# NeSC-IV/sage-icp

Measured on AMD Instinct MI355X. Metric: ICP frames/sec (120k-pt scan vs 1M-pt map), higher is better.
Workload: dtype f64

## Files before the change

### include/sageicp.h

```cpp
#ifndef SAGEICP_H_
#define SAGEICP_H_

#include <stddef.h>
#include <stdint.h>

#ifdef __cplusplus
extern "C" {
#endif

#define SAGEICP_OK 0
#define SAGEICP_ERR_INVALID (-1)
#define SAGEICP_ERR_NO_DEVICE (-2)
#define SAGEICP_ERR_HIP (-3)
#define SAGEICP_ERR_RCCL (-4)
#define SAGEICP_ERR_CAPACITY (-5)

typedef struct sageicp_map sageicp_map;
typedef struct sageicp_frame sageicp_frame;
typedef struct sageicp_comm sageicp_comm;

#define SAGEICP_ABI_VERSION 4

typedef struct sageicp_stats {
    int32_t iterations;
// ... 140 lines not shown
int sageicp_cluster_emission_order(const uint32_t *sizes, uint64_t n, uint32_t *order_out);

int sageicp_deskew_scan(const double *frame_xyzl, const double *timestamps, uint64_t n,
                        const double start_pose[7], const double finish_pose[7],
                        double *out_xyzl, int device);

typedef struct sageicp_pipeline sageicp_pipeline;
typedef struct sageicp_pipeline_config {
    double voxel_size_map, max_range, min_range, label_max_range, local_map_range;
    int basic_points_per_voxel, critical_points_per_voxel;
    const int *basic_parts_labels;
    int n_basic_parts_labels;
    double min_motion_th, initial_threshold, sem_th;
    int n_groups;
    const int *group_label_counts;
    const int *group_labels;
    const double *group_voxel_size;
    int device;
    int map_update_on_device;
} sageicp_pipeline_config;

sageicp_pipeline *sageicp_pipeline_create(const sageicp_pipeline_config *config);
void sageicp_pipeline_destroy(sageicp_pipeline *p);
int sageicp_pipeline_register_frame(sageicp_pipeline *p, const double *frame_xyzl, uint64_t n,
                                    double pose_out[7], double *icp_seconds, double *total_seconds,
                                    uint64_t *n_source, sageicp_stats *stats );
int sageicp_pipeline_prefetch(sageicp_pipeline *p, const double *next_frame_xyzl, uint64_t n);
int sageicp_pipeline_prefetch_wait(sageicp_pipeline *p);
int sageicp_pipeline_prefetch_cancel(sageicp_pipeline *p);
int sageicp_pipeline_set_dynamic_vehicle_filter(sageicp_pipeline *p, int enable, double dy_th,
                                                int dynamic_vehicle_voxid, const int *landmark_labels,
                                                int n_landmark);
int sageicp_pipeline_dynamic_filter_info(const sageicp_pipeline *p, sageicp_dynfilter_info *info);
int sageicp_pipeline_set_deskew(sageicp_pipeline *p, int enable);
int sageicp_pipeline_register_frame_timestamps(sageicp_pipeline *p, const double *frame_xyzl,
                                               const double *timestamps, uint64_t n, double pose_out[7],
                                               double *icp_seconds, double *total_seconds, uint64_t *n_source,
                                               sageicp_stats *stats );
int sageicp_pipeline_deskew_info(const sageicp_pipeline *p, int *applied, double delta_out[6]);

#define SAGEICP_DTYPE_FLOAT32 1
#define SAGEICP_DTYPE_FLOAT64 2
#define SAGEICP_DTYPE_UINT8 3
#define SAGEICP_DTYPE_INT32 4
#define SAGEICP_DTYPE_INT64 5
typedef struct sageicp_device_frame {
    const void *xyz;
    uint64_t xyz_stride;
    int32_t xyz_dtype;
    int32_t label_dtype;
    const void *label;
    uint64_t label_stride;
    uint64_t n;
} sageicp_device_frame;
int sageicp_pipeline_register_frame_device(sageicp_pipeline *p, const sageicp_device_frame *frame,
                                           const double *timestamps ,
                                           void *stream , double pose_out[7],
                                           double *icp_seconds, double *total_seconds, uint64_t *n_source,
                                           sageicp_stats *stats );
sageicp_frame *sageicp_frame_from_device(const sageicp_map *map, const sageicp_device_frame *frame,
                                         void *stream );

typedef struct sageicp_device_points {
    void *xyz;
    uint64_t xyz_stride;
    int32_t xyz_dtype;
    int32_t label_dtype;
    void *label;
    uint64_t label_stride;
    uint64_t cap;
} sageicp_device_points;
int sageicp_pipeline_source(const sageicp_pipeline *p, double *out_xyzl, uint64_t cap, uint64_t *n_out);
int sageicp_pipeline_source_device(const sageicp_pipeline *p, const sageicp_device_points *dst,
                                   void *stream , uint64_t *n_out);
int sageicp_map_pointcloud_device(const sageicp_map *m, const sageicp_device_points *dst,
                                  void *stream , uint64_t *n_out);
int sageicp_get_correspondences_device(const sageicp_map *map, const sageicp_device_frame *frame,
                                       const double pose[7] ,
                                       double max_correspondence_distance, double sem_th,
                                       const sageicp_device_points *src_out ,
                                       const sageicp_device_points *tgt_out ,
                                       int64_t *query_idx_out , uint64_t idx_cap,
                                       void *stream , uint64_t *n_out);

typedef struct sageicp_quality {
    double fitness, rmse, step_norm;
    double sum_r2, sum_w, sum_w_r2;
    double step[6];
    double JTr[6];
    double JTJ[36];
    double info[36];
    double covariance[36];
    double covariance_pose[36];
    double class_sum_r2[256];
    double other_sum_r2;
    uint64_t n_queries, n_pairs;
    uint64_t pairs_same_label, pairs_unlabelled, pairs_cross_label;
    uint64_t other_queries, other_pairs;
    uint32_t class_queries[256];
    uint32_t class_pairs[256];
    int32_t valid, covariance_valid;
} sageicp_quality;
int sageicp_registration_quality(const sageicp_map *map, const double *xyzl, uint64_t n,
                                 const double pose[7] , double max_correspondence_distance,
                                 double kernel, double sem_th, sageicp_quality *out);
int sageicp_registration_quality_device(const sageicp_map *map, const sageicp_device_frame *frame,
                                        const double pose[7] , double max_correspondence_distance,
                                        double kernel, double sem_th, void *stream ,
                                        sageicp_quality *out);
int sageicp_pipeline_set_quality(sageicp_pipeline *p, int enable);
int sageicp_pipeline_quality(const sageicp_pipeline *p, sageicp_quality *out);

typedef struct sageicp_pose_score {
    double score;
    double fitness, rmse, step_norm;
    double sum_r2, sum_w, sum_w_r2;
    double step[6], JTr[6], JTJ[36];
    uint64_t n_queries, n_pairs, pairs_same_label, pairs_unlabelled, pairs_cross_label;
    int32_t valid, step_valid;
} sageicp_pose_score;
int sageicp_score_poses(const sageicp_map *map, const double *xyzl, uint64_t n,
                        const double *poses , uint64_t k,
                        double max_correspondence_distance, double kernel, double sem_th,
                        sageicp_pose_score *out );
int sageicp_score_poses_device(const sageicp_map *map, const sageicp_device_frame *frame,
                               const double *poses , uint64_t k,
                               double max_correspondence_distance, double kernel, double sem_th,
                               void *stream , sageicp_pose_score *out);

typedef struct sageicp_relocalize_params {
    double xy_extent, xy_step, z_extent, z_step;
    double yaw_extent, yaw_step;
    uint32_t refine_top, reserved;
    double max_correspondence_distance, kernel, sem_th;
} sageicp_relocalize_params;
typedef struct sageicp_relocalize_info {
    uint64_t candidates, best_candidate;
    double best_candidate_score;
    uint32_t refined, winner_rank;
    int32_t iterations, converged;
    double us_score, us_refine, us_wall;
} sageicp_relocalize_info;
int sageicp_relocalize_candidates(const double prior[7], const sageicp_relocalize_params *params,
                                  double *poses_out , uint64_t cap, uint64_t *k_out);
int sageicp_relocalize(const sageicp_map *map, const double *xyzl, uint64_t n, const double prior[7],
                       const sageicp_relocalize_params *params, double pose_out[7],
                       sageicp_quality *quality_out , sageicp_relocalize_info *info );
int sageicp_relocalize_device(const sageicp_map *map, const sageicp_device_frame *frame, const double prior[7],
                              const sageicp_relocalize_params *params, void *stream, double pose_out[7],
                              sageicp_quality *quality_out, sageicp_relocalize_info *info);

int sageicp_pipeline_reinitialize(sageicp_pipeline *p);
uint64_t sageicp_pipeline_num_poses(const sageicp_pipeline *p);
int sageicp_pipeline_pose(const sageicp_pipeline *p, uint64_t index, double pose_out[7]);
const sageicp_map *sageicp_pipeline_local_map(const sageicp_pipeline *p);

typedef struct sageicp_occupancy_params {
    double bounds[3][2];
    int32_t occ_h, occ_w;
    double overlap_th;
} sageicp_occupancy_params;
typedef struct sageicp_key_frame_info {
    int32_t enabled;
    int32_t is_key_frame;
    double overlap;
    uint64_t key_frame_index;
// ... 93 lines not shown
```

### sage-icp_amd/__init__.py

```python
import ctypes as C
import os
import sys

import numpy as np

_HERE = os.path.dirname(os.path.abspath(__file__))
SQNORM3_ORDER = 0 if os.environ.get("SAGE_SQNORM3_ORDER", "2") == "0" else 2
if os.environ.get("SAGE_SQNORM3_ORDER", "2") not in ("0", "2"):
    import warnings
    warnings.warn("SAGE_SQNORM3_ORDER=%r: only the builds 0 and 2 exist — using 2" % os.environ["SAGE_SQNORM3_ORDER"])
LIB_PATH = os.path.join(_HERE, "libsageicp_hip.v0.so" if SQNORM3_ORDER == 0 else "libsageicp_hip.so")
if os.environ.get("SAGEICP_VARIANT_LIB"):
    LIB_PATH = os.path.abspath(os.environ["SAGEICP_VARIANT_LIB"])

_dp = C.POINTER(C.c_double)
_u64p = C.POINTER(C.c_uint64)
_i64p = C.POINTER(C.c_int64)
_u8p = C.POINTER(C.c_uint8)

ABI_VERSION = 4
ERR_INVALID, ERR_NO_DEVICE, ERR_HIP, ERR_RCCL, ERR_CAPACITY = -1, -2, -3, -4, -5
UNIQUE_ID_BYTES = 128
P2P_HANDLE_BYTES = 64

# ... 192 lines not shown
def occupancy_params(bounds=KEY_FRAME_BOUNDS, occ_size=KEY_FRAME_OCC_SIZE, overlap=KEY_FRAME_OVERLAP):
    b = [[float(v) for v in ax] for ax in bounds]
    if len(b) != 3 or any(len(ax) != 2 for ax in b):
        raise ValueError("bounds are ((x_lo, x_hi), (y_lo, y_hi), (z_lo, z_hi))")
    h, w = (int(v) for v in occ_size)
    p = OccupancyParams()
    for a in range(3):
        p.bounds[a][0], p.bounds[a][1] = b[a]
    p.occ_h, p.occ_w, p.overlap_th = h, w, float(overlap)
    return p


KITTI_VOXEL_LABELS = [[40, 44, 48, 49], [50, 51, 52], [70, 72], [60, 71, 80, 81, 99], [0],
                      [10, 11, 13, 15, 16, 18, 20]]
KITTI_VOXEL_SIZE = [0.6, 1.0, 0.9, 0.8, 1.0, 0.6]


def make_pipeline_config(voxel_size_map=0.8, max_range=100.0, min_range=5.0, label_max_range=50.0,
                         local_map_range=100.0, basic=20, critical=20,
                         basic_parts_labels=(40, 44, 48, 49, 50, 70, 72), min_motion_th=0.1,
                         initial_threshold=2.0, sem_th=0.05, voxel_labels=None, voxel_size=None,
                         device=0, map_update_on_device=True, dynamic_vehicle_filter=False,
                         dynamic_vehicle_filter_th=0.5, dynamic_vehicle_voxid=5, dynamic_remove_lankmark=(44, 48),
                         deskew=False):
    voxel_labels = KITTI_VOXEL_LABELS if voxel_labels is None else voxel_labels
    voxel_size = KITTI_VOXEL_SIZE if voxel_size is None else voxel_size
    assert len(voxel_labels) == len(voxel_size)
    keep = {}
    keep["basic"] = (C.c_int * len(basic_parts_labels))(*basic_parts_labels)
    keep["counts"] = (C.c_int * len(voxel_labels))(*[len(g) for g in voxel_labels])
    flat = [l for g in voxel_labels for l in g]
    keep["labels"] = (C.c_int * len(flat))(*flat)
    keep["sizes"] = (C.c_double * len(voxel_size))(*voxel_size)
    cfg = PipelineConfig(voxel_size_map, max_range, min_range, label_max_range, local_map_range,
                         basic, critical, keep["basic"], len(basic_parts_labels), min_motion_th,
                         initial_threshold, sem_th, len(voxel_labels), keep["counts"],
                         keep["labels"], keep["sizes"], device, 1 if map_update_on_device else 0)
    cfg._keep = keep
    cfg._dynamic = dict(enable=bool(dynamic_vehicle_filter), dy_th=float(dynamic_vehicle_filter_th),
                        voxid=int(dynamic_vehicle_voxid), landmarks=tuple(dynamic_remove_lankmark))
    cfg._deskew = bool(deskew)
    return cfg


_SIGNATURES = [
    ("sageicp_abi_version", C.c_int, []),
    ("sageicp_last_error", C.c_char_p, []),
    ("sageicp_device_count", C.c_int, []),
    ("sageicp_set_profiling", None, [C.c_int]),
    ("sageicp_set_counting", None, [C.c_int]),
    ("sageicp_reload_env", None, []),
    ("sageicp_map_loop_status", C.c_int, [C.c_void_p, C.c_void_p]),
    ("sageicp_set_downsample_order", None, [C.c_int]),
    ("sageicp_robin_iteration_order", C.c_int, [C.c_void_p, C.c_uint64, C.c_void_p]),
    ("sageicp_robin_sweep", C.c_int, [C.c_void_p, C.c_uint64, C.c_void_p, C.c_int, C.c_void_p, _u64p, C.c_void_p, _u64p]),
    ("sageicp_map_create", C.c_void_p,
     [C.c_double, C.c_double, C.c_int, C.c_int, C.POINTER(C.c_int), C.c_int, C.c_int]),
    ("sageicp_map_destroy", None, [C.c_void_p]),
    ("sageicp_map_set_devices", C.c_int, [C.c_void_p, C.POINTER(C.c_int), C.c_int]),
    ("sageicp_map_num_devices", C.c_int, [C.c_void_p]),
    ("sageicp_map_set_reference_order", C.c_int, [C.c_void_p, C.c_int]),
    ("sageicp_map_reference_order", C.c_int, [C.c_void_p]),
    ("sageicp_map_clone", C.c_void_p, [C.c_void_p]),
    ("sageicp_map_clear", C.c_int, [C.c_void_p]),
    ("sageicp_map_empty", C.c_int, [C.c_void_p]),
    ("sageicp_map_size", C.c_uint64, [C.c_void_p]),
    ("sageicp_map_num_voxels", C.c_uint64, [C.c_void_p]),
    ("sageicp_map_add_points", C.c_int, [C.c_void_p, _dp, C.c_uint64]),
    ("sageicp_map_remove_far", C.c_int, [C.c_void_p, _dp]),
    ("sageicp_map_update", C.c_int, [C.c_void_p, _dp, C.c_uint64, _dp]),
    ("sageicp_map_update_pose", C.c_int, [C.c_void_p, _dp, C.c_uint64, _dp]),
    ("sageicp_map_update_pose_device", C.c_int, [C.c_void_p, _dp, C.c_uint64, _dp]),
    ("sageicp_map_pointcloud", C.c_uint64, [C.c_void_p, _dp, C.c_uint64]),
    ("sageicp_map_resident", C.c_int, [C.c_void_p]),
    ("sageicp_map_point_slots", C.c_uint64, [C.c_void_p]),
    ("sageicp_voxel_hash", C.c_uint32, [C.c_int32, C.c_int32, C.c_int32]),
    ("sageicp_map_table_stats", C.c_int, [C.c_void_p, _u64p]),
    ("sageicp_map_sync", C.c_int, [C.c_void_p]),
    ("sageicp_get_correspondences", C.c_int,
     [C.c_void_p, _dp, C.c_uint64, C.c_double, C.c_double, _dp, _dp, _u64p, _i64p]),
    ("sageicp_get_correspondences_device", C.c_int,
     [C.c_void_p, C.POINTER(DeviceFrame), _dp, C.c_double, C.c_double, C.POINTER(DevicePoints), C.POINTER(DevicePoints),
      C.c_void_p, C.c_uint64, C.c_void_p, _u64p]),
    ("sageicp_registration_quality", C.c_int,
     [C.c_void_p, _dp, C.c_uint64, _dp, C.c_double, C.c_double, C.c_double, C.POINTER(Quality)]),
    ("sageicp_registration_quality_device", C.c_int,
     [C.c_void_p, C.POINTER(DeviceFrame), _dp, C.c_double, C.c_double, C.c_double, C.c_void_p, C.POINTER(Quality)]),
    ("sageicp_pipeline_set_quality", C.c_int, [C.c_void_p, C.c_int]),
    ("sageicp_pipeline_quality", C.c_int, [C.c_void_p, C.POINTER(Quality)]),
    ("sageicp_score_poses", C.c_int,
     [C.c_void_p, _dp, C.c_uint64, _dp, C.c_uint64, C.c_double, C.c_double, C.c_double, C.c_void_p]),
    ("sageicp_score_poses_device", C.c_int,
     [C.c_void_p, C.POINTER(DeviceFrame), _dp, C.c_uint64, C.c_double, C.c_double, C.c_double, C.c_void_p, C.c_void_p]),
    ("sageicp_relocalize_candidates", C.c_int, [_dp, C.POINTER(RelocalizeParams), _dp, C.c_uint64, _u64p]),
    ("sageicp_relocalize", C.c_int,
     [C.c_void_p, _dp, C.c_uint64, _dp, C.POINTER(RelocalizeParams), _dp, C.POINTER(Quality), C.POINTER(RelocalizeInfo)]),
    ("sageicp_relocalize_device", C.c_int,
     [C.c_void_p, C.POINTER(DeviceFrame), _dp, C.POINTER(RelocalizeParams), C.c_void_p, _dp, C.POINTER(Quality),
      C.POINTER(RelocalizeInfo)]),
    ("sageicp_align_clouds", C.c_int, [_dp, _dp, C.c_uint64, C.c_double, _dp, _dp, _dp, C.c_int]),
    ("sageicp_transform_points", C.c_int, [_dp, _dp, C.c_uint64, C.c_int]),
    ("sageicp_register_frame", C.c_int,
     [C.c_void_p, _dp, C.c_uint64, _dp, C.c_double, C.c_double, C.c_double, _dp,
      C.POINTER(Stats)]),
    ("sageicp_frame_upload", C.c_void_p, [C.c_void_p, _dp, C.c_uint64]),
    ("sageicp_frame_destroy", None, [C.c_void_p]),
    ("sageicp_register_frame_resident", C.c_int,
     [C.c_void_p, C.c_void_p, _dp, C.c_double, C.c_double, C.c_double, C.c_void_p, _dp,
      C.POINTER(Stats)]),
    ("sageicp_comm_unique_id", C.c_int, [_u8p]),
    ("sageicp_comm_create", C.c_void_p, [_u8p, C.c_int, C.c_int, C.c_int]),
    ("sageicp_comm_create_local", C.c_void_p, [C.c_int, C.c_int, C.c_int]),
    ("sageicp_comm_p2p_export", C.c_int, [C.c_void_p, C.POINTER(C.c_uint8)]),
    ("sageicp_comm_p2p_connect", C.c_int, [C.c_void_p, C.POINTER(C.c_uint8)]),
    ("sageicp_comm_p2p_enable", C.c_int, [C.c_void_p, C.c_int]),
    ("sageicp_comm_p2p_enabled", C.c_int, [C.c_void_p]),
    ("sageicp_comm_describe", C.c_int, [C.c_void_p, C.POINTER(CommInfo)]),
    ("sageicp_comm_destroy", None, [C.c_void_p]),
    ("sageicp_preprocess", C.c_int,
     [_dp, C.c_uint64, C.c_double, C.c_double, C.c_double, _dp, _u64p, C.c_int]),
    ("sageicp_voxel_downsample", C.c_int,
     [_dp, C.c_uint64, C.c_int, C.POINTER(C.c_int), C.POINTER(C.c_int), C.POINTER(C.c_double),
      C.c_double, _dp, _u64p, C.c_int]),
    ("sageicp_preprocess_dynamic", C.c_int,
     [_dp, C.c_uint64, C.c_double, C.c_double, C.c_double, C.c_double, C.POINTER(C.c_int), C.c_int,
      C.POINTER(C.c_int), C.c_int, _dp, _u64p, C.POINTER(DynFilterInfo), C.c_int]),
    ("sageicp_cluster_emission_order", C.c_int, [C.c_void_p, C.c_uint64, C.c_void_p]),
    ("sageicp_pipeline_set_dynamic_vehicle_filter", C.c_int,
     [C.c_void_p, C.c_int, C.c_double, C.c_int, C.POINTER(C.c_int), C.c_int]),
    ("sageicp_pipeline_dynamic_filter_info", C.c_int, [C.c_void_p, C.POINTER(DynFilterInfo)]),
    ("sageicp_deskew_scan", C.c_int, [_dp, _dp, C.c_uint64, _dp, _dp, _dp, C.c_int]),
    ("sageicp_pipeline_set_deskew", C.c_int, [C.c_void_p, C.c_int]),
    ("sageicp_pipeline_register_frame_timestamps", C.c_int,
     [C.c_void_p, _dp, _dp, C.c_uint64, _dp, _dp, _dp, _u64p, C.POINTER(Stats)]),
    ("sageicp_pipeline_deskew_info", C.c_int, [C.c_void_p, C.POINTER(C.c_int), _dp]),
    ("sageicp_pipeline_register_frame_device", C.c_int,
     [C.c_void_p, C.POINTER(DeviceFrame), C.c_void_p, C.c_void_p, _dp, _dp, _dp, _u64p, C.POINTER(Stats)]),
    ("sageicp_frame_from_device", C.c_void_p, [C.c_void_p, C.POINTER(DeviceFrame), C.c_void_p]),
    ("sageicp_pipeline_source", C.c_int, [C.c_void_p, _dp, C.c_uint64, _u64p]),
    ("sageicp_pipeline_source_device", C.c_int, [C.c_void_p, C.POINTER(DevicePoints), C.c_void_p, _u64p]),
    ("sageicp_map_pointcloud_device", C.c_int, [C.c_void_p, C.POINTER(DevicePoints), C.c_void_p, _u64p]),
    ("sageicp_pipeline_set_key_frames", C.c_int, [C.c_void_p, C.c_int, C.POINTER(OccupancyParams)]),
    ("sageicp_pipeline_key_frame_reset", C.c_int, [C.c_void_p]),
    ("sageicp_pipeline_key_frame_info", C.c_int, [C.c_void_p, C.POINTER(KeyFrameInfo)]),
    ("sageicp_pipeline_key_frame_grid", C.c_int, [C.c_void_p, C.c_void_p, C.c_uint64]),
    ("sageicp_pipeline_key_frame_grid_device", C.c_int, [C.c_void_p, C.c_void_p, C.c_uint64, C.c_void_p]),
    ("sageicp_occupancy_grid", C.c_int, [_dp, C.c_uint64, _dp, C.POINTER(OccupancyParams), C.c_void_p, C.c_int]),
    ("sageicp_occupancy_grid_device", C.c_int,
     [C.POINTER(DeviceFrame), _dp, C.POINTER(OccupancyParams), C.c_void_p, C.c_void_p]),
    ("sageicp_pipeline_register_frame_msg", C.c_int,
     [C.c_void_p, C.c_void_p, C.c_uint64, C.c_uint64, C.POINTER(MsgLayout), _dp, _dp, _dp, _u64p, C.POINTER(Stats)]),
    ("sageicp_pipeline_register_frame_msg_device", C.c_int,
     [C.c_void_p, C.c_void_p, C.c_uint64, C.c_uint64, C.POINTER(MsgLayout), C.c_void_p, _dp, _dp, _dp, _u64p,
      C.POINTER(Stats)]),
    ("sageicp_msg_output_fields", C.c_uint32, [C.POINTER(MsgField), C.c_uint32]),
    ("sageicp_pipeline_source_msg", C.c_int, [C.c_void_p, C.POINTER(MsgColors), C.c_void_p, C.c_uint64, _u64p]),
    ("sageicp_pipeline_source_msg_device", C.c_int,
     [C.c_void_p, C.POINTER(MsgColors), C.c_void_p, C.c_uint64, C.c_void_p, _u64p]),
    ("sageicp_map_pointcloud_msg", C.c_int, [C.c_void_p, C.POINTER(MsgColors), C.c_void_p, C.c_uint64, _u64p]),
    ("sageicp_map_pointcloud_msg_device", C.c_int,
     [C.c_void_p, C.POINTER(MsgColors), C.c_void_p, C.c_uint64, C.c_void_p, _u64p]),
    ("sageicp_map_set_archive", C.c_int, [C.c_void_p, C.c_int, C.c_uint64]),
    ("sageicp_map_archive_info", C.c_int, [C.c_void_p, C.POINTER(ArchiveInfo)]),
    ("sageicp_map_archive_clear", C.c_int, [C.c_void_p]),
    ("sageicp_map_archive_voxels", C.c_int, [C.c_void_p, C.c_uint64, C.c_void_p, C.c_uint64, _u64p]),
    ("sageicp_map_archive_rows", C.c_int, [C.c_void_p, C.c_int, C.c_uint64, _dp, C.c_uint64, _u64p]),
# ... 656 lines not shown
            _check(lib().sageicp_relocalize_device(self._h, C.byref(f), pr, C.byref(params), stream,
                                                   pose.ctypes.data_as(_dp), C.byref(q), C.byref(info)))
            return pose, q, info.as_dict()
        if labels is not None:
            raise ValueError("labels= is for a frame that is a torch tensor on a GPU")
        pts, fp = _d(pts)
        _check(lib().sageicp_relocalize(self._h, fp, pts.reshape(-1, 4).shape[0], pr, C.byref(params),
                                        pose.ctypes.data_as(_dp), C.byref(q), C.byref(info)))
        return pose, q, info.as_dict()

    def _correspondences_device(self, pts, max_dist, th, with_index, labels, pose, dtype):
        f, stream = _device_rows(DeviceFrame, pts, labels, self.device, _FRAME_WORDS)
        pp = None
        if pose is not None:
            pose_a, pp = _d(pose)
            if pose_a.size != 7:
                raise ValueError("a pose is (qx, qy, qz, qw, tx, ty, tz)")
        import torch
        dt = torch.float64 if dtype is None else dtype
        if dt not in (torch.float32, torch.float64):
            raise ValueError("dtype= is torch.float32 or torch.float64, not %s" % (dt,))
        n = int(f.n)
        src = torch.empty((n, 4), dtype=dt, device=pts.device)
        tgt = torch.empty((n, 4), dtype=dt, device=pts.device)
        idx = torch.empty(n, dtype=torch.int64, device=pts.device) if with_index else None
        ds, _ = _device_rows(DevicePoints, src, None, self.device, _OUT_WORDS, distinct=True)
        dg, _ = _device_rows(DevicePoints, tgt, None, self.device, _OUT_WORDS, distinct=True)
        nout = C.c_uint64(0)
        _check(lib().sageicp_get_correspondences_device(
            self._h, C.byref(f), pp, max_dist, th, C.byref(ds), C.byref(dg),
            (idx.data_ptr() or None) if with_index else None, n, stream, C.byref(nout)))
        k = nout.value
        return (src[:k], tgt[:k], idx[:k]) if with_index else (src[:k], tgt[:k])


def _relocalize_params(xy, z, yaw, refine_top=0, max_correspondence_distance=0.0, kernel=1.0, sem_th=0.0):
    p = RelocalizeParams()
    (p.xy_extent, p.xy_step), (p.z_extent, p.z_step), (p.yaw_extent, p.yaw_step) = xy, z, yaw
    p.refine_top = refine_top
    p.max_correspondence_distance, p.kernel, p.sem_th = max_correspondence_distance, kernel, sem_th
    return p


def relocalize_candidates(prior, xy=(0, 0), z=(0, 0), yaw=(0, 0), cap=None):
    prior_a, pr = _d(prior)
    if prior_a.size != 7:
        raise ValueError("a pose is (qx, qy, qz, qw, tx, ty, tz)")
    params = _relocalize_params(xy, z, yaw)
    k = C.c_uint64(0)
    if cap is None:
        _check(lib().sageicp_relocalize_candidates(pr, C.byref(params), None, 0, C.byref(k)))
    rows = k.value if cap is None else int(cap)
    out = np.empty((rows, 7))
    _check(lib().sageicp_relocalize_candidates(pr, C.byref(params), out.ctypes.data_as(_dp), rows, C.byref(k)))
    return out if cap is None else (out[:min(rows, k.value)], k.value)


def register_frame(frame, voxel_map, initial_guess, max_correspondence_distance, kernel, sem_th,
                   comm=None, return_stats=False):
    init, ip = _d(initial_guess)
    out = np.empty(7)
    st = Stats()
    if isinstance(frame, Frame):
        _check(lib().sageicp_register_frame_resident(
            voxel_map._h, frame._h, ip, max_correspondence_distance, kernel, sem_th,
            comm._h if comm is not None else None, out.ctypes.data_as(_dp), C.byref(st)))
    else:
        if comm is not None:
            raise ValueError("sharded registration needs a resident Frame")
        pts, pp = _d(frame)
        _check(lib().sageicp_register_frame(
            voxel_map._h, pp, pts.reshape(-1, 4).shape[0], ip, max_correspondence_distance,
            kernel, sem_th, out.ctypes.data_as(_dp), C.byref(st)))
    return (out, st) if return_stats else out


def transform_points(pose, pts, device=0):
    T, tp = _d(pose)
    out = np.array(pts, dtype=np.float64, order="C", copy=True).reshape(-1, 4)
    _check(lib().sageicp_transform_points(tp, out.ctypes.data_as(_dp), out.shape[0], device))
    return out


def occupancy_grid(frame, bounds=KEY_FRAME_BOUNDS, occ_size=KEY_FRAME_OCC_SIZE, pose=None, device=0, labels=None):
    params = occupancy_params(bounds, occ_size, 0.0)
    out = np.zeros((params.occ_h, params.occ_w), dtype=np.uint8)
    pp = None
    if pose is not None:
        pose_a, pp = _d(pose)
        if pose_a.size != 7:
            raise ValueError("a pose is (qx, qy, qz, qw, tx, ty, tz)")
    if _is_device_tensor(frame):
        f, stream = _device_rows(DeviceFrame, frame, labels, frame.device.index, _FRAME_WORDS)
        _check(lib().sageicp_occupancy_grid_device(C.byref(f), pp, C.byref(params), out.ctypes.data_as(C.c_void_p),
                                                   stream))
        return out
    if labels is not None:
        raise ValueError("labels= is for a frame that is a torch tensor on a GPU")
    pts, fp = _d(frame)
    _check(lib().sageicp_occupancy_grid(fp, pts.reshape(-1, 4).shape[0], pp, C.byref(params),
                                        out.ctypes.data_as(C.c_void_p), device))
    return out


def align_clouds(src, tgt, kernel, device=0):
    src, sp = _d(src)
    tgt, gp = _d(tgt)
    T = np.empty(7)
    JTJ = np.empty(36)
    JTr = np.empty(6)
    _check(lib().sageicp_align_clouds(sp, gp, src.reshape(-1, 4).shape[0], kernel,
                                      T.ctypes.data_as(_dp), JTJ.ctypes.data_as(_dp),
                                      JTr.ctypes.data_as(_dp), device))
    return T, JTJ.reshape(6, 6), JTr


class SageICP:

    def __init__(self, config=None, **kw):
        self.config = config if config is not None else make_pipeline_config(**kw)
        self._h = lib().sageicp_pipeline_create(C.byref(self.config))
        if not self._h:
            raise SageIcpError(ERR_INVALID, (lib().sageicp_last_error() or b"").decode())
        self._deskew_on = False
        dyn = getattr(self.config, "_dynamic", None)
        if dyn and dyn["enable"]:
            self.set_dynamic_vehicle_filter(True, dyn["dy_th"], dyn["voxid"], dyn["landmarks"])
        if getattr(self.config, "_deskew", False):
            self.set_deskew(True)

    def set_deskew(self, enable=True):
        _check(lib().sageicp_pipeline_set_deskew(self._h, 1 if enable else 0))
        self._deskew_on = bool(enable)
        if enable:
            self._announced = ()

    def deskew_info(self):
        applied = C.c_int(0)
        delta = np.zeros(6)
        _check(lib().sageicp_pipeline_deskew_info(self._h, C.byref(applied), delta.ctypes.data_as(_dp)))
        return bool(applied.value), delta

    def set_dynamic_vehicle_filter(self, enable=True, dy_th=0.5, voxid=5, landmark_labels=(44, 48)):
        lm = (C.c_int * max(len(landmark_labels), 1))(*landmark_labels)
        _check(lib().sageicp_pipeline_set_dynamic_vehicle_filter(self._h, 1 if enable else 0, dy_th, voxid, lm,
                                                                 len(landmark_labels)))

    def set_quality(self, enable=True):
        _check(lib().sageicp_pipeline_set_quality(self._h, 1 if enable else 0))

    def quality(self):
        q = Quality()
        _check(lib().sageicp_pipeline_quality(self._h, C.byref(q)))
        return q

    def set_key_frames(self, enable=True, bounds=KEY_FRAME_BOUNDS, occ_size=KEY_FRAME_OCC_SIZE, overlap=KEY_FRAME_OVERLAP):
        params = occupancy_params(bounds, occ_size, overlap) if enable else None
        _check(lib().sageicp_pipeline_set_key_frames(self._h, 1 if enable else 0,
                                                     C.byref(params) if params is not None else None))
        self._occ_size = (params.occ_h, params.occ_w) if enable else None

    def key_frame_info(self):
        info = KeyFrameInfo()
        _check(lib().sageicp_pipeline_key_frame_info(self._h, C.byref(info)))
        return info.as_dict()

# ... 313 lines not shown
```

### sage-icp_amd/build.py

```python
import concurrent.futures
import hashlib
import os
import subprocess

HERE = os.path.dirname(os.path.abspath(__file__))
SOURCES = ["csrc/kernels.hip", "csrc/sort.hip", "csrc/preprocess.hip", "csrc/dyn_filter.hip", "csrc/deskew.hip",
           "csrc/ingest.hip", "csrc/egress.hip", "csrc/msg.hip", "csrc/keyframe.hip", "csrc/map_update.hip",
           "csrc/map_device.hip", "csrc/capi_run.hip", "csrc/prep.hip", "csrc/capi.hip", "csrc/capi_pipeline.hip",
           "csrc/capi_outputs.hip", "csrc/caller_mem.hip", "csrc/correspond.hip", "csrc/quality.hip", "csrc/score.hip",
           "csrc/capi_query.hip", "csrc/capi_relocalize.hip", "csrc/archive.hip", "csrc/capi_archive.hip"]
HEADERS = ["csrc/kernels.h", "csrc/dev_buffer.h", "csrc/sageicp_types.h", "csrc/se3_math.h", "csrc/host_map.hpp", "csrc/pipeline.hpp", "csrc/map_update.h", "csrc/egress.h", "csrc/msg.h", "csrc/metrics.hpp", "csrc/robin_order.hpp", "csrc/capi_internal.h", "csrc/prep.h", "csrc/prefetch.h", "csrc/dyn_rules.h", "csrc/probes.h", "csrc/icp_body.h", "csrc/row_shift.h", "csrc/fin_kernel.h", "csrc/loop_kernel.h", "csrc/loop_deal.h", "csrc/caller_mem.h", "csrc/outputs.h", "csrc/map_device.h", "csrc/replay_pool.h", "csrc/correspond.h", "csrc/quality.h", "csrc/score.h", "csrc/accept.h", "csrc/archive.h", "csrc/query.h",
           "../include/sageicp.h"]
OUT = os.path.join(HERE, "libsageicp_hip.so")
OBJ_DIR = os.path.join(HERE, "build")

FLAGS = ["--offload-arch=gfx950", "-O3", "-std=c++17", "-fPIC", "-ffp-contract=off",
         "-Wall", "-Wextra"]


def _stamp(extra):
    h = hashlib.sha1(" ".join(FLAGS + list(extra)).encode())
    for f in HEADERS:
        with open(os.path.join(HERE, f), "rb") as fh:
            h.update(fh.read())
    return h.hexdigest()[:16]


def needs_build():
    if not os.path.exists(OUT):
        return True
    t = os.path.getmtime(OUT)
    return any(os.path.getmtime(os.path.join(HERE, f)) > t for f in SOURCES + HEADERS)


def _prune(keep, newest=6):
    import shutil
    dirs = [os.path.join(OBJ_DIR, d) for d in os.listdir(OBJ_DIR)]
    dirs = sorted((d for d in dirs if os.path.isdir(d) and d != keep), key=os.path.getmtime, reverse=True)
    for d in dirs[newest - 1:]:
        shutil.rmtree(d, ignore_errors=True)


def build(force=False, verbose=False, out=OUT, defines=(), jobs=None):
    if not force and out == OUT and not defines and not needs_build():
        return out
    hipcc = os.environ.get("HIPCC", "/opt/rocm/bin/hipcc")
    extra = ["-D" + d for d in defines]
    tag = _stamp(extra)
    odir = os.path.join(OBJ_DIR, tag)
    os.makedirs(odir, exist_ok=True)
    _prune(keep=odir)

    def compile_one(src):
        path = os.path.join(HERE, src)
        obj = os.path.join(odir, os.path.basename(src) + ".o")
        if os.path.exists(obj) and os.path.getmtime(obj) >= os.path.getmtime(path):
            return obj
        cmd = [hipcc] + FLAGS + extra + ["-c", path, "-o", obj]
        if verbose:
            print(" ".join(cmd))
        subprocess.check_call(cmd)
        return obj

    with concurrent.futures.ThreadPoolExecutor(max_workers=jobs or min(len(SOURCES), os.cpu_count() or 1)) as ex:
        objs = list(ex.map(compile_one, SOURCES))
    cmd = [hipcc, "--offload-arch=gfx950", "-shared", "-fPIC"] + objs + ["-o", out, "-ldl", "-lpthread"]
    if verbose:
        print(" ".join(cmd))
    subprocess.check_call(cmd)
    return out


def build_sqnorm3_variant(force=False, verbose=False):
    out = os.path.join(HERE, "libsageicp_hip.v0.so")
    if not force and os.path.exists(out):
        t = os.path.getmtime(out)
        if not any(os.path.getmtime(os.path.join(HERE, f)) > t for f in SOURCES + HEADERS):
            return out
    return build(force=True, verbose=verbose, out=out, defines=("SAGE_SQNORM3_ORDER=0",))


PROBE_DEFINES = ("SAGE_NN_TIMING", "SAGE_LOOP_TIMING", "SAGE_GN_TIMING", "SAGE_ICP_DELAY_PROBE", "SAGE_LOOP_INGRID")


def compile_probe_variants(jobs=None):
    hipcc = os.environ.get("HIPCC", "/opt/rocm/bin/hipcc")
    src = os.path.join(HERE, "csrc/kernels.hip")

    def one(d):
        r = subprocess.run([hipcc] + FLAGS + ["-D" + d, "--cuda-device-only", "-c", src, "-o", os.devnull],
                           capture_output=True, text=True)
        return d, (r.stderr if r.returncode else "")

    with concurrent.futures.ThreadPoolExecutor(max_workers=jobs or min(len(PROBE_DEFINES), os.cpu_count() or 1)) as ex:
# ... 9 lines not shown
```

### sage-icp_amd/csrc/capi_internal.h

```cpp
#pragma once

#include <dlfcn.h>
#include <hip/hip_runtime.h>
#include <rccl/rccl.h>

#include <atomic>
#include <chrono>
#include <cmath>
#include <cstdio>
#include <cstdlib>
#include <cfloat>
#include <limits>
#include <memory>
#include <cstring>
#include <map>
#include <array>
#include <string>
#include <utility>
#include <vector>

#include "../../include/sageicp.h"
#include "dev_buffer.h"
#include "dyn_rules.h"
#include "host_map.hpp"
// ... 39 lines not shown
inline int icp_lw(uint64_t n, bool sparse_voxels) {
    const int e = env_int("SAGEICP_LW", -1);
    if (e >= 0) return e > 4 ? 4 : e;
    if (n >= (sparse_voxels ? 150000u : 400000u)) return 1;
    if (n >= (sparse_voxels ? 60000u : 110000u)) return 2;
    if (n >= (sparse_voxels ? 4096u : 20000u)) return 3;
    return 4;
}


inline int fail(int code, const std::string &msg) {
    g_err = msg;
    return code;
}

#define HIPCHK(expr)                                                                      \
    do {                                                                                  \
        hipError_t _e = (expr);                                                           \
        if (_e != hipSuccess)                                                             \
            return fail(SAGEICP_ERR_HIP, std::string(#expr) + ": " + hipGetErrorString(_e)); \
    } while (0)

inline int require_device() {
    int count = 0;
    if (hipGetDeviceCount(&count) != hipSuccess || count <= 0)
        return fail(SAGEICP_ERR_NO_DEVICE, "no HIP device visible (gfx950 required; no CPU fallback)");
    return SAGEICP_OK;
}
inline int require_device(int device) {
    if (int rc = require_device()) return rc;
    if (device < 0 || device >= sageicp_device_count()) return fail(SAGEICP_ERR_INVALID, "device ordinal out of range");
    return SAGEICP_OK;
}

inline int stream_after_caller(OwnedEvent &ev, hipStream_t caller, hipStream_t ours) {
    if (!ev) HIPCHK(ev.create(hipEventDisableTiming));
    HIPCHK(hipEventRecord(ev.get(), caller));
    HIPCHK(hipStreamWaitEvent(ours, ev.get(), 0));
    return SAGEICP_OK;
}

inline bool finite_n(const double *v, uint64_t n) {
    for (uint64_t i = 0; i < n; ++i)
        if (!std::isfinite(v[i])) return false;
    return true;
}

inline double now_us() {
    using namespace std::chrono;
    return duration<double, std::micro>(steady_clock::now().time_since_epoch()).count();
}

constexpr int kChunkMax = 16;

struct Scratch {
    int device = -1;
    OwnedStream stream;
    DevBuf<Point4> d_frame, d_tgt;
    DevBuf<int32_t> d_nn;
    DevBuf<Point4> d_sorted;
    DevBuf<uint32_t> d_keys, d_vals;
    DevBuf<unsigned char> d_sort_temp;
    size_t sort_cap = 0;
    DevBuf<uint32_t> d_rows;
    DevBuf<uint2> d_prev;
    DevBuf<uint32_t> d_work;
    DevBuf<double> d_partials;
    DevBuf<long long> d_acc;
    DevBuf<LoopShared> d_loop;
    unsigned long long go_word = 0;
    OwnedStream stream2;
    std::vector<uint32_t> cu_mask;
    OwnedEvent ev_solve;
    unsigned long long loop_epoch = 0;
    int num_cus = 0;
    int cu_share_i = 0, cu_share_k = 1;
    int loop_cooldown = 0;
    int loop_derate = 0;
    uint64_t calls_single_launch = 0, calls_per_iteration = 0, calls_chained = 0;
    uint32_t loop_timeouts = 0;
    int last_fallback = 0;
    DevBuf<unsigned long long> d_cand;
    DevBuf<IcpState> d_state;
    PinnedBuf<IcpState> h_state;
    PinnedBuf<IcpProgress, hipHostMallocMapped | hipHostMallocCoherent> h_prog;
    IcpProgress *d_prog = nullptr;
    std::vector<OwnedEvent> events;
    DevBuf<int32_t> d_by_query;
    DevBuf<uint32_t> d_corr_counts;
    DevBuf<unsigned long long> d_corr_words;
    PinnedBuf<unsigned long long> h_corr_words;
    DevBuf<double> d_qual_slabs;
    DevBuf<QualityRaw> d_qual_raw;
    PinnedBuf<QualityRaw> h_qual_raw;
    DevBuf<Point4> d_score_frame, d_score_rows;
    DevBuf<int32_t> d_score_by_query;
    DevBuf<double> d_score_slabs;
    DevBuf<ScorePose> d_score_poses;
    PinnedBuf<ScorePose> h_score_poses;
    DevBuf<ScoreRaw> d_score_raw;
    PinnedBuf<ScoreRaw> h_score_raw;

    ~Scratch() { wait(); }
    void wait() const {
        if (!stream) return;
        (void)hipSetDevice(device);
        (void)hipStreamSynchronize(stream.get());
        if (stream2) (void)hipStreamSynchronize(stream2.get());
    }

    int init(int dev) {
        if (stream) return SAGEICP_OK;
        if (int rc = require_device(dev)) return rc;
        device = dev;
        HIPCHK(hipSetDevice(device));
        {
            int cus = 0;
            if (hipDeviceGetAttribute(&cus, hipDeviceAttributeMultiprocessorCount, device) == hipSuccess) num_cus = cus;
        }
        if (cu_share_k <= 1) {
            if (const char *e = env_cached("SAGEICP_CU_SHARE")) {
                int i = 0, k = 1;
                if (std::sscanf(e, "%d/%d", &i, &k) == 2 && k >= 1 && k <= 16 && i >= 0 && i < k) {
                    cu_share_i = i;
                    cu_share_k = k;
                }
            }
        }
        if (cu_share_k > 1 && num_cus >= 8 * cu_share_k) {
            const int per = num_cus / cu_share_k, lo = cu_share_i * per;
            std::vector<uint32_t> mask((num_cus + 31) / 32, 0u);
            for (int c = lo; c < lo + per; ++c) mask[c / 32] |= 1u << (c % 32);
            HIPCHK(stream.create(static_cast<uint32_t>(mask.size()), mask.data()));
            cu_mask = mask;
            num_cus = per;
        } else {
            cu_share_i = 0;
            cu_share_k = 1;
            HIPCHK(stream.create());
        }
        HIPCHK(d_state.reserve(1));
        HIPCHK(d_acc.reserve(kAccReplicas * kAccWords));
        HIPCHK(d_loop.reserve(1));
        HIPCHK(hipMemset(d_loop.data(), 0, sizeof(LoopShared)));

        HIPCHK(h_state.reserve(1));
        HIPCHK(h_prog.reserve(1));
        HIPCHK(hipHostGetDevicePointer(reinterpret_cast<void **>(&d_prog), h_prog.data(), 0));
        return SAGEICP_OK;
    }
    int loop_streams() {
        if (stream2) return SAGEICP_OK;
        HIPCHK(hipSetDevice(device));
        if (!cu_mask.empty()) HIPCHK(stream2.create(static_cast<uint32_t>(cu_mask.size()), cu_mask.data()));
        else {
            int least = 0, greatest = 0;
            (void)hipDeviceGetStreamPriorityRange(&least, &greatest);
            if (stream2.create(greatest) != hipSuccess) {
                (void)hipGetLastError();
                HIPCHK(stream2.create());
            }
        }
        HIPCHK(ev_solve.create(hipEventDisableTiming));
        return SAGEICP_OK;
    }
    int reserve_frame(size_t n) {
        if (n > d_frame.capacity()) HIPCHK(d_frame.reserve(n + n / 4 + 1024));
        return SAGEICP_OK;
    }
    int reserve_tgt(size_t n) {
        if (n > d_tgt.capacity()) HIPCHK(d_tgt.reserve(n + n / 4 + 1024));
        return SAGEICP_OK;
    }
    int reserve_nn(size_t n) {
        if (n > d_nn.capacity()) HIPCHK(d_nn.reserve(n + n / 4 + 1024));
        return SAGEICP_OK;
    }
    int reserve_sort(size_t n) {
        if (n <= sort_cap) return SAGEICP_OK;
        sort_cap = 0;
        const size_t cap = n + n / 4 + 1024;
        HIPCHK(d_sorted.reserve(cap));
        HIPCHK(d_rows.reserve(cap * kRowWords));
        HIPCHK(d_prev.reserve(cap));
#ifdef SAGE_NN_TIMING
        HIPCHK(d_work.reserve(cap));
#endif
        HIPCHK(d_cand.reserve(2 * cap));
        HIPCHK(d_keys.reserve(2 * cap));
        HIPCHK(d_vals.reserve(2 * cap));
        HIPCHK(d_sort_temp.reserve(sort_temp_bytes(static_cast<int>(cap))));
        sort_cap = cap;
        return SAGEICP_OK;
    }
    int reserve_correspond(size_t n) {
        if (n > d_by_query.capacity()) HIPCHK(d_by_query.reserve(n + n / 4 + 1024));
        const size_t words = 2 * static_cast<size_t>(correspond_blocks(static_cast<int>(n)));
        if (words > d_corr_counts.capacity()) HIPCHK(d_corr_counts.reserve(words + words / 4 + 16));
        if (!d_corr_words) HIPCHK(d_corr_words.reserve(2));
        if (!h_corr_words) HIPCHK(h_corr_words.reserve(2));
        return SAGEICP_OK;
    }
    int reserve_quality(size_t n) {
        if (n > d_by_query.capacity()) HIPCHK(d_by_query.reserve(n + n / 4 + 1024));
        if (!d_qual_slabs) HIPCHK(d_qual_slabs.reserve(kQualSlabDoubles));
        if (!d_qual_raw) HIPCHK(d_qual_raw.reserve(1));
        if (!h_qual_raw) HIPCHK(h_qual_raw.reserve(1));
        return SAGEICP_OK;
    }
    int reserve_score_frame(size_t n) {
        if (n > d_score_frame.capacity()) HIPCHK(d_score_frame.reserve(n + n / 4 + 1024));
        return SAGEICP_OK;
    }
    int reserve_score(size_t n, size_t kc) {
        const size_t rows = n * kc, slabs = score_slab_doubles(static_cast<int>(n), static_cast<uint32_t>(kc));
        if (rows > d_score_rows.capacity()) HIPCHK(d_score_rows.reserve(rows + rows / 4 + 1024));
        if (rows > d_score_by_query.capacity()) HIPCHK(d_score_by_query.reserve(rows + rows / 4 + 1024));
        if (slabs > d_score_slabs.capacity()) HIPCHK(d_score_slabs.reserve(slabs + slabs / 4 + 1024));
        if (kc > d_score_poses.capacity()) HIPCHK(d_score_poses.reserve(kc + kc / 4 + 16));
        if (kc > h_score_poses.capacity()) HIPCHK(h_score_poses.reserve(kc + kc / 4 + 16));
        if (kc > d_score_raw.capacity()) HIPCHK(d_score_raw.reserve(kc + kc / 4 + 16));
        if (kc > h_score_raw.capacity()) HIPCHK(h_score_raw.reserve(kc + kc / 4 + 16));
        return SAGEICP_OK;
    }
    int reserve_partials(size_t blocks) {
        if (blocks > d_partials.capacity() / kNumSums) HIPCHK(d_partials.reserve((blocks + blocks / 4 + 256) * kNumSums));
        return SAGEICP_OK;
    }
    int reserve_events(size_t iterations) {
        while (events.size() < 5 * iterations) {
            OwnedEvent e;
// ... 9 lines not shown

#include "prep.h"

using namespace sageicp;

#include "caller_mem.h"
#include "map_device.h"
#include "archive.h"
#include "outputs.h"

struct sageicp_map {
    HostMap host;
    int device = 0;
    Scratch sc;
    sageicp_impl::MapDevice dev;
    sageicp_impl::OutputBuffers out;
    sageicp_impl::MapArchive arc;
    std::vector<sageicp_map *> replicas;
    std::vector<struct sageicp_comm *> ranks;
    bool replicas_diverged = false;

    bool resident() const { return dev.authority(); }
    bool empty() const { return counts().voxels == 0; }
    sageicp_impl::MapCounts counts() const {
        const bool on_device = dev.authority();
        const MapCounters &c = dev.ctr;
        sageicp_impl::MapCounts n;
        n.points = on_device ? c.total_points : host.total_points;
        n.voxels = on_device ? c.num_voxels : host.num_voxels;
        n.units_hi = on_device ? c.units_hi : host.units_hi;
        n.table_capacity = on_device ? dev.d_table.capacity() : host.table.size();
        n.used_slots = on_device ? c.used_slots : host.num_voxels;
        return n;
    }
    ~sageicp_map() { sc.wait(); }
};

inline sageicp_map &internal(const sageicp_map *m) { return *const_cast<sageicp_map *>(m); }

struct sageicp_frame {
    int device = 0;
    DevBuf<Point4> d;
    uint64_t n = 0;
};

struct sageicp_comm {
    ncclComm_t comm = nullptr;
    int rank = 0, nranks = 1, device = 0;
    bool p2p = false;
    bool poisoned = false;
    P2pBlock *my_block = nullptr;
    P2pBlock *blocks[kMaxRanks] = {};
    DevBuf<unsigned long long> d_exchanges;
    bool peer_mapped = false;
    bool device_shared = false;
};

namespace sageicp_impl {
struct Rccl {
    void *h = nullptr;
    ncclResult_t (*GetUniqueId)(ncclUniqueId *) = nullptr;
    ncclResult_t (*CommInitRank)(ncclComm_t *, int, ncclUniqueId, int) = nullptr;
    ncclResult_t (*CommDestroy)(ncclComm_t) = nullptr;
    ncclResult_t (*AllReduce)(const void *, void *, size_t, ncclDataType_t, ncclRedOp_t, ncclComm_t,
                              hipStream_t) = nullptr;
    const char *(*GetErrorString)(ncclResult_t) = nullptr;
    ncclResult_t (*CommCount)(const ncclComm_t, int *) = nullptr;
    ncclResult_t (*CommUserRank)(const ncclComm_t, int *) = nullptr;
};
extern Rccl g_rccl;
int load_rccl();
int register_resident(sageicp_map &m, const Point4 *d_frame, uint64_t n, int device, const double init[7],
                      double max_dist, double kernel, double sem_th, sageicp_comm *comm, double pose_out[7],
                      sageicp_stats *stats);
int refresh_mirror(sageicp_map &m);
int ensure_host(sageicp_map &m);
int device_update(sageicp_map &m, const double *xyzl, uint64_t n, const double pose[7], const Point4 *d_points = nullptr);
bool all_finite(const double *xyzl, uint64_t n);
void host_remove_far(sageicp_map &m, const double origin[3]);
void identity_pose(double T[7]);
void fill_state(IcpState *st, const double init[7]);
double accept_threshold(double max_dist);
bool sparse_voxels(const sageicp_map &m);
bool wants_filter(const sageicp_map &m, uint64_t n, double sem_th);
IcpParams icp_params(const sageicp_map &m, const Point4 *d_queries, uint64_t n, double sem_th, int lw, int acc_shift);
int run_icp(sageicp_map &m, const Point4 *d_frame, uint64_t n, const double init[7], double max_dist, double kernel,
            double sem_th, sageicp_comm *comm, double out[7], sageicp_stats *stats, double us_upload, double t_begin);
int device_update_all(sageicp_map &m, const double *xyzl, uint64_t n, const double pose[7], const Point4 *d_points);
int register_sharded(sageicp_map &m, const double *h_frame, const Point4 *d_frame, uint64_t n, const double init[7],
                     double max_dist, double kernel, double sem_th, double pose_out[7], sageicp_stats *stats, double t0);
}
using namespace sageicp_impl;
```

### sage-icp_amd/csrc/capi_query.hip

```cpp
#include "query.h"

namespace sageicp_impl {

int QueryCall::stage(const FrameSource &src, Point4 *d_dst) {
    if (src.kind == FrameSource::kHostRows) {
        HIPCHK(hipMemcpyAsync(d_dst, src.rows, src.n * sizeof(Point4), hipMemcpyHostToDevice, stream()));
        return SAGEICP_OK;
    }
    if (src.kind != FrameSource::kDeviceFrame)
        return fail(SAGEICP_ERR_INVALID, std::string(who_) + ": host rows or a device frame");
    if (int rc = stream_after_caller(m.out.ev_caller, src.stream, stream())) return rc;
    launch_ingest(ingest_args(*src.frame), d_dst, stream());
    HIPCHK(hipGetLastError());
    return SAGEICP_OK;
}

int QueryCall::stage(const Point4 *d_rows, uint64_t n, Point4 *d_dst) {
    HIPCHK(hipMemcpyAsync(d_dst, d_rows, n * sizeof(Point4), hipMemcpyDeviceToDevice, stream()));
    return SAGEICP_OK;
}

int QueryCall::move(Point4 *d_rows, uint64_t n, const double *pose) {
    double I[7];
    identity_pose(I);
    fill_state(sc.h_state.data(), pose ? pose : I);
    HIPCHK(hipMemcpyAsync(sc.d_state.data(), sc.h_state.data(), sizeof(IcpState), hipMemcpyHostToDevice, stream()));
    if (pose) launch_tf(d_rows, static_cast<int>(n), sc.d_state.data(), stream());
    HIPCHK(hipGetLastError());
    return SAGEICP_OK;
}

int QueryCall::sort_and_search(const Point4 *d_rows, uint64_t n, double sem_th, bool read_verdict) {
    HIPCHK(sort_frame(d_rows, sc.d_sorted.data(), static_cast<int>(n), sc.d_state.data(), false, false,
                      m.host.voxel_size, sc.d_keys.data(), sc.d_vals.data(), sc.d_sort_temp.data(),
                      sc.d_sort_temp.capacity(), stream()));
    if (read_verdict) {
        HIPCHK(hipMemcpyAsync(sc.h_state.data(), sc.d_state.data(), sizeof(IcpState), hipMemcpyDeviceToHost, stream()));
        if (int rc = wait()) return rc;
        if (sc.h_state.data()->bad_input) return refuse_non_finite(who_, noun_);
    }
    const int lw = icp_lw(n, sparse_voxels(m));
    if (int rc = m.dev.ensure_cand(wants_filter(m, n, sem_th), stream())) return rc;
    const IcpParams ip = icp_params(m, sc.d_sorted.data(), n, sem_th, lw, 0);
    launch_rows(ip, stream());
    launch_icp(ip, lw, false, stream());
    HIPCHK(hipGetLastError());
    return SAGEICP_OK;
}

CorrespondArgs QueryCall::answers(uint64_t n, double max_dist, int32_t *d_by_query) const {
    CorrespondArgs a{};
    a.n = static_cast<int>(n);
    a.sorted = sc.d_sorted.data();
    a.perm = sc.d_vals.data() + n;
    a.nn = sc.d_nn.data();
    a.pts = m.dev.search_view().pts;
    a.accept_r2 = accept_threshold(max_dist);
    a.by_query = d_by_query;
    return a;
}

int QueryCall::accept(uint64_t n, double max_dist, int32_t *d_by_query) {
    launch_corr_flag(answers(n, max_dist, d_by_query), stream());
    HIPCHK(hipGetLastError());
    return SAGEICP_OK;
}

int refuse_non_finite(const char *who, const char *noun) {
    return fail(SAGEICP_ERR_INVALID,
                std::string(who) + ": a coordinate or label of a " + noun + " is not finite (NaN / Inf)");
}

int check_host_rows(const char *who, const double *xyzl, uint64_t n) {
    if (n && !xyzl) return fail(SAGEICP_ERR_INVALID, std::string(who) + ": xyzl is NULL");
    if (n > kMaxQueries) return fail(SAGEICP_ERR_INVALID, std::string(who) + ": too many rows (2^26 - 4 max)");
    if (!all_finite(xyzl, n)) return refuse_non_finite(who, "row");
    return SAGEICP_OK;
}

int check_device_source(const char *who, const sageicp_map *map, const sageicp_device_frame *frame, void *stream) {
    if (!frame) return fail(SAGEICP_ERR_INVALID, std::string(who) + ": frame is NULL");
    if (int rc = check_frame_layout(frame)) return rc;
    if (int rc = check_device_frame(frame, nullptr, stream, map->device)) return rc;
    return check_stream(stream, map->device);
}

static_assert(sizeof(sageicp_quality) == 5464, "sageicp_quality: doubles first, no padding (include/sageicp.h)");
static_assert(kQualClasses == 256, "the class tables of sageicp_quality");

constexpr double kQualPivotBound = 1.0 / 67108864.0;

bool quality_solve(const double JTJ[36], const double JTr[6], double sum_w_r2, uint64_t n_pairs, QualitySolve *o) {
    if (n_pairs < 3) return false;
    const double np = static_cast<double>(n_pairs);
    double L[6][6] = {};
    for (int j = 0; j < 6; ++j) {
        double d = JTJ[j * 6 + j];
        for (int k = 0; k < j; ++k) d -= L[j][k] * L[j][k];
        if (!(d > kQualPivotBound * JTJ[j * 6 + j]) || !std::isfinite(d)) return false;
        L[j][j] = std::sqrt(d);
        for (int i = j + 1; i < 6; ++i) {
            double v = JTJ[i * 6 + j];
            for (int k = 0; k < j; ++k) v -= L[i][k] * L[j][k];
            L[i][j] = v / L[j][j];
        }
    }
    double Li[6][6] = {};
    for (int j = 0; j < 6; ++j) {
        Li[j][j] = 1.0 / L[j][j];
        for (int i = j + 1; i < 6; ++i) {
            double v = 0.0;
            for (int k = j; k < i; ++k) v -= L[i][k] * Li[k][j];
            Li[i][j] = v / L[i][i];
        }
    }
    for (int i = 0; i < 6; ++i)
        for (int j = 0; j <= i; ++j) {
            double v = 0.0;
// ... 95 lines not shown
                          c.stream()));
    if ((rc = c.wait())) return rc;
    quality_finish(*sc.h_qual_raw.data(), n, pose, out);
    return SAGEICP_OK;
}

int quality_of_device_rows(sageicp_map &m, const Point4 *d_rows, uint64_t n, const double *pose, double max_dist,
                           double kernel, double sem_th, sageicp_quality *out) {
    QueryCall c(m, "RegistrationQuality");
    if (int rc = c.sc.reserve_frame(n)) return rc;
    if (int rc = c.stage(d_rows, n, c.sc.d_frame.data())) return rc;
    return quality_of_staged_rows(c, n, pose, max_dist, kernel, sem_th, out);
}

static int check_quality_args(const sageicp_map *map, const double *pose, double kernel, const sageicp_quality *out) {
    if (!map) return fail(SAGEICP_ERR_INVALID, "RegistrationQuality: map is NULL");
    if (!out) return fail(SAGEICP_ERR_INVALID, "RegistrationQuality: out is NULL");
    if (pose && !finite_n(pose, 7)) return fail(SAGEICP_ERR_INVALID, "RegistrationQuality: the pose is not finite");
    if (!(std::isfinite(kernel) && kernel > 0.0))
        return fail(SAGEICP_ERR_INVALID, "RegistrationQuality: kernel must be finite and above 0");
    return SAGEICP_OK;
}

static int registration_quality(const sageicp_map *map, const FrameSource &src, const double *pose, double max_dist,
                                double kernel, double sem_th, sageicp_quality *out) {
    std::memset(out, 0, sizeof(*out));
    sageicp_map &m = internal(map);
    if (src.n == 0 || m.empty()) return SAGEICP_OK;
    int rc = refresh_mirror(m);
    if (rc) return rc;
    QueryCall c(m, "RegistrationQuality");
    if ((rc = m.sc.reserve_frame(src.n))) return rc;
    if ((rc = c.stage(src, m.sc.d_frame.data()))) return rc;
    return quality_of_staged_rows(c, src.n, pose, max_dist, kernel, sem_th, out);
}

}

extern "C" {

int sageicp_get_correspondences(const sageicp_map *map, const double *q, uint64_t n, double max_dist,
                                double sem_th, double *src_out, double *tgt_out, uint64_t *n_out,
                                int64_t *query_idx_out) {
    if (!map || !n_out || (n && (!q || !src_out || !tgt_out)))
        return fail(SAGEICP_ERR_INVALID, "null argument");
    if (n > kMaxQueries) return fail(SAGEICP_ERR_INVALID, "too many queries (2^26 - 4 max)");
    *n_out = 0;
    if (!all_finite(q, n)) return refuse_non_finite("GetCorrespondences", "query");
    sageicp_map &m = internal(map);
    int rc = ensure_host(m);
    if (rc) return rc;
    if ((rc = refresh_mirror(m))) return rc;
    if (n == 0 || m.empty()) return SAGEICP_OK;
    QueryCall c(m, "GetCorrespondences", "query");
    Scratch &sc = m.sc;
    if ((rc = sc.reserve_frame(n))) return rc;
    if ((rc = sc.reserve_nn(n))) return rc;
    if ((rc = sc.reserve_sort(n))) return rc;
    if ((rc = c.stage(FrameSource::host_rows(q, n), sc.d_frame.data()))) return rc;
    if ((rc = c.move(sc.d_frame.data(), n, nullptr))) return rc;
    if ((rc = c.sort_and_search(sc.d_frame.data(), n, sem_th,  false))) return rc;
    std::vector<int32_t> idx(n);
    std::vector<uint32_t> perm(n);
    HIPCHK(hipMemcpyAsync(idx.data(), sc.d_nn.data(), n * sizeof(int32_t), hipMemcpyDeviceToHost, c.stream()));
    HIPCHK(hipMemcpyAsync(perm.data(), sc.d_vals.data() + n, n * sizeof(uint32_t), hipMemcpyDeviceToHost, c.stream()));
    if ((rc = c.wait())) return rc;
    std::vector<int32_t> by_query(n);
    for (uint64_t i = 0; i < n; ++i) by_query[perm[i]] = idx[i];
    uint64_t k = 0;
    for (uint64_t i = 0; i < n; ++i) {
        if (by_query[i] < 0) continue;
        const Point4 &t = m.host.pts[by_query[i]];
        const double dx = t.x - q[4 * i], dy = t.y - q[4 * i + 1], dz = t.z - q[4 * i + 2];
        if (!(std::sqrt(SAGE_SQNORM3_ACCEPT(dx * dx, dy * dy, dz * dz)) < max_dist)) continue;
        std::memcpy(src_out + 4 * k, q + 4 * i, 32);
        std::memcpy(tgt_out + 4 * k, &t, 32);
        if (query_idx_out) query_idx_out[k] = static_cast<int64_t>(i);
        ++k;
    }
    *n_out = k;
    return SAGEICP_OK;
}

int sageicp_get_correspondences_device(const sageicp_map *map, const sageicp_device_frame *frame, const double pose[7],
                                       double max_dist, double sem_th, const sageicp_device_points *src_out,
                                       const sageicp_device_points *tgt_out, int64_t *query_idx_out, uint64_t idx_cap,
                                       void *stream, uint64_t *n_out) {
    if (!map || !frame || !n_out) return fail(SAGEICP_ERR_INVALID, "null argument");
    int rc = check_frame_layout(frame);
    if (!rc && src_out) rc = check_points_layout(src_out);
    if (!rc && tgt_out) rc = check_points_layout(tgt_out);
    if (rc) return rc;
    if (pose && !finite_n(pose, 7)) return fail(SAGEICP_ERR_INVALID, "GetCorrespondences: the pose is not finite");
    {
        const uint64_t caps[3] = {src_out ? src_out->cap : 0, tgt_out ? tgt_out->cap : 0, idx_cap};
        const bool given[3] = {src_out != nullptr, tgt_out != nullptr, query_idx_out != nullptr};
        for (int a = 0; a < 3; ++a)
            for (int b = a + 1; b < 3; ++b)
                if (given[a] && given[b] && caps[a] != caps[b])
                    return fail(SAGEICP_ERR_INVALID, "GetCorrespondences: src_out->cap, tgt_out->cap and idx_cap of the "
                                                     "destinations given must be equal");
    }
    if (reinterpret_cast<uintptr_t>(query_idx_out) % 8)
        return fail(SAGEICP_ERR_INVALID, "GetCorrespondences: query_idx_out must be 8-byte aligned");
    CallerExtent ext[5];
    int n_ext = 0;
    int first_of_tgt = 0, first_of_idx = 0;
    if (src_out) n_ext += points_extents(*src_out, ext + n_ext);
    first_of_tgt = n_ext;
    if (tgt_out) n_ext += points_extents(*tgt_out, ext + n_ext);
    first_of_idx = n_ext;
    if (query_idx_out && idx_cap) {
        const char *p = reinterpret_cast<const char *>(query_idx_out);
        ext[n_ext++] = {p, p + idx_cap * sizeof(int64_t)};
    }
    for (int a = 0; a < n_ext; ++a)
        for (int b = a + 1; b < n_ext; ++b) {
            const bool same = (b < first_of_tgt) || (a >= first_of_tgt && b < first_of_idx);
            if (!same && ext[a].overlaps(ext[b]))
                return fail(SAGEICP_ERR_INVALID, "GetCorrespondences: src_out, tgt_out and query_idx_out must not overlap "
                                                 "each other");
        }
    if ((rc = check_device_frame(frame, nullptr, stream, map->device))) return rc;
    if (src_out && (rc = check_device_points(src_out, stream, map->device))) return rc;
    if (tgt_out && (rc = check_device_points(tgt_out, stream, map->device))) return rc;
    if (query_idx_out && idx_cap) {
        if ((rc = require_device())) return rc;
        if ((rc = check_extent(query_idx_out, idx_cap * sizeof(int64_t), map->device, "GetCorrespondences: query_idx_out")))
            return rc;
    }
    if ((rc = check_stream(stream, map->device))) return rc;
    sageicp_map &m = internal(map);
    const uint64_t n = frame->n;
    if (n == 0 || m.empty()) {
        *n_out = 0;
        return SAGEICP_OK;
    }
    if ((rc = refresh_mirror(m))) return rc;
    QueryCall c(m, "GetCorrespondences", "query");
    Scratch &sc = m.sc;
    if ((rc = sc.reserve_frame(n))) return rc;
    if ((rc = sc.reserve_nn(n))) return rc;
    if ((rc = sc.reserve_sort(n))) return rc;
    if ((rc = sc.reserve_correspond(n))) return rc;
    if ((rc = c.stage(FrameSource::device_frame(frame, nullptr, static_cast<hipStream_t>(stream)), sc.d_frame.data())))
        return rc;
    if ((rc = c.move(sc.d_frame.data(), n, pose))) return rc;
    if ((rc = c.sort_and_search(sc.d_frame.data(), n, sem_th))) return rc;
    HIPCHK(hipMemsetAsync(sc.d_corr_words.data(), 0, 2 * sizeof(unsigned long long), c.stream()));
    int *flags = reinterpret_cast<int *>(sc.d_corr_words.data() + 1);
    CorrespondArgs a = c.answers(n, max_dist, sc.d_by_query.data());
    a.frame = sc.d_frame.data();
    a.counts = sc.d_corr_counts.data();
    a.total = sc.d_corr_words.data();
    a.has_src = src_out != nullptr;
    a.has_tgt = tgt_out != nullptr;
    if (src_out) a.src = egress_args(*src_out, flags);
    if (tgt_out) a.tgt = egress_args(*tgt_out, flags);
    a.idx = reinterpret_cast<long long *>(query_idx_out);
    a.idx_cap = idx_cap;
    launch_correspond(a, c.stream());
    HIPCHK(hipGetLastError());
    unsigned long long *h_words = sc.h_corr_words.data();
    HIPCHK(hipMemcpyAsync(h_words, sc.d_corr_words.data(), 2 * sizeof(unsigned long long), hipMemcpyDeviceToHost,
                          c.stream()));
    if ((rc = c.wait())) return rc;
// ... 27 lines not shown
```

### sage-icp_amd/csrc/capi_run.hip

```cpp
#include "capi_internal.h"
#include "accept.h"

#include <condition_variable>
#include <mutex>
#include <thread>

namespace sageicp_impl {

Rccl g_rccl;
static std::mutex g_rccl_mu;


int load_rccl() {
    std::lock_guard<std::mutex> lk(g_rccl_mu);
    if (g_rccl.h) return SAGEICP_OK;
    const char *names[] = {"librccl.so.1", "librccl.so", "/opt/rocm/lib/librccl.so.1"};
    void *h = nullptr;
    for (const char *n : names) {
        h = dlopen(n, RTLD_NOW | RTLD_NOLOAD | RTLD_GLOBAL);
        if (h) break;
    }
    for (int i = 0; i < 3 && !h; ++i) h = dlopen(names[i], RTLD_NOW | RTLD_GLOBAL);
    if (!h) return fail(SAGEICP_ERR_RCCL, std::string("cannot load librccl: ") + dlerror());
    g_rccl.GetUniqueId = reinterpret_cast<decltype(g_rccl.GetUniqueId)>(dlsym(h, "ncclGetUniqueId"));
// ... 116 lines not shown
    if (mode == 0 || n == 0 || sc.num_cus < 8) return false;
    const bool sparse = sparse_voxels(m);
    const bool filter = wants_filter(m, n, sem_th);
    const uint64_t cus = static_cast<uint64_t>(sc.num_cus);
    const int env_nw = std::min(kLoopMaxWavesHost, std::max(0, env_int("SAGEICP_LOOP_WAVES", 0)));
    const int env_gpw = std::max(0, env_int("SAGEICP_LOOP_GPW", 0));
    auto groups_at = [n](int l) { return (n + (64u >> l) - 1) / (64u >> l); };
    auto slots = [&](int k) {
        const uint64_t a = static_cast<uint64_t>(k) * cus * 15 / 16;
        int less = 0;
        for (int sh = 1; sh < sc.cu_share_k; sh *= 2) ++less;
        return (less > 0 && k > less) ? std::min(a, static_cast<uint64_t>(k - less) * cus) : a;
    };
    auto round32 = [](uint64_t w) { return std::max<uint64_t>(32, (w + 31) / 32 * 32); };
    auto countable = [](uint64_t wgs, uint64_t gpw, int lw) {
        return wgs / kLoopReplicas <= 255 && (wgs / kLoopReplicas) * gpw * ((64u >> lw) / 4u) <= 8192;
    };
    auto one_pass = [&](int lw, int nw, LoopPlan *pl) {
        const uint64_t wgs = round32((groups_at(lw) + nw - 1) / nw);
        const size_t lds = loop_lds_bytes(lw, nw, nw);
        const int k = loop_wgs_per_cu(sc, lw, filter, nw, lds);
        if (k < 1 || wgs + 32ull * static_cast<uint64_t>(sc.loop_derate) > slots(k) || !countable(wgs, nw, lw)) return false;
        *pl = LoopPlan{lw, nw, nw, static_cast<int>(wgs), filter};
        return true;
    };
    auto multi_pass = [&](int lw, LoopPlan *pl) {
        const uint64_t groups = groups_at(lw);
        int best = -1;
        const int order[] = {4, 8, 7, 6, 5, 3, 2, 1};
        for (int nw : order) {
            if (env_nw && nw != env_nw) continue;
            if (!env_nw && nw < 4) continue;
            for (int k = SAGE_LOOP_OCC / ((nw + 3) / 4); k >= 1; --k) {
                if (static_cast<uint64_t>(k) * cus < 34) break;
                uint64_t cap = slots(k) / 32 * 32;
                cap = cap > 32ull * static_cast<uint64_t>(sc.loop_derate) ? cap - 32ull * static_cast<uint64_t>(sc.loop_derate) : 0;
                if (cap < 32) continue;
                if (const int e = env_int("SAGEICP_LOOP_MAX_WGS", 0)) cap = std::min<uint64_t>(cap, static_cast<uint64_t>(e) / 32 * 32);
                uint64_t gpw = env_gpw ? static_cast<uint64_t>(env_gpw) : (groups + cap - 1) / cap;
                const uint64_t wgs = env_gpw ? round32((groups + gpw - 1) / gpw) : std::min(cap, round32(groups));
                if (wgs > cap) continue;
                if (!env_gpw) gpw = (groups + wgs - 1) / wgs;
                const size_t lds = loop_lds_bytes(lw, nw, static_cast<int>(gpw));
                if (lds > 160 * 1024 || !countable(wgs, gpw, lw)) continue;
                if (loop_wgs_per_cu(sc, lw, filter, nw, lds) < k) continue;
                if (k * nw > best) {
                    best = k * nw;
                    *pl = LoopPlan{lw, nw, static_cast<int>(gpw), static_cast<int>(wgs), filter};
                }
                break;
            }
        }
        return best > 0;
    };
    const int forced = env_int("SAGEICP_LW", -1);
    int lw = forced >= 0 ? std::min(forced, 4) : icp_lw(n, sparse);
    if (lw < 1) return false;
    if (forced < 0 && !env_gpw) {
        const uint64_t few = 15 * cus;
        if (lw < 3 && groups_at(3) <= few) lw = 3;
        if (lw == 3 && !sparse && groups_at(4) <= few) lw = 4;
        const uint64_t resident_waves = 4ull * SAGE_LOOP_OCC * cus * 15 / 16;
        while (lw > 2 && groups_at(lw) > resident_waves * 4 / 5) --lw;
    }
    const bool dbg = env_int("SAGEICP_LOOP_DEBUG", 0) != 0;
    bool ok = !env_gpw && one_pass(lw, env_nw ? env_nw : 4, out);
    if (!ok) ok = multi_pass(lw, out);
    if (dbg) {
        if (ok)
            std::fprintf(stderr, "sageicp: one-launch loop for %llu queries: %d lanes/query, %d workgroups of %d waves, <= %d units of %d queries each, "
                                 "%zu B of LDS (%d workgroups per CU by the occupancy query, %d CUs)\n",
                         static_cast<unsigned long long>(n), 1 << out->lw, out->wgs, out->nw,
                         out->gpw, 64 >> out->lw, loop_lds_bytes(out->lw, out->nw, out->gpw),
                         loop_wgs_per_cu(sc, out->lw, filter, out->nw, loop_lds_bytes(out->lw, out->nw, out->gpw)), sc.num_cus);
        else
            std::fprintf(stderr, "sageicp: %llu queries at %d lanes/query do not fit the one-launch loop (7 waves x 4 workgroups "
                                 "of 36 KB per CU by the occupancy query: %d)\n",
                         static_cast<unsigned long long>(n), 1 << lw,
                         loop_wgs_per_cu(sc, lw, filter, 7, 36 * 1024));
    }
    return ok;
}

struct Attempt {
    int acc_shift = 0;
    int restarts = 0;
    bool no_loop = false;
    bool no_chain = false;
};

struct IcpCall {
    sageicp_map &m;
    const Point4 *d_frame;
    uint64_t n;
    const double *init;
    double max_dist, kernel, sem_th;
    sageicp_comm *comm;
    Scratch &sc;
    hipStream_t s;
    bool p2p, polled, prof, prof2, counting;
    int max_it;
    P2pParams xp;

    int constants(bool want_stats) {
        prof = g_profiling != 0;
        prof2 = g_profiling >= 2;
        p2p = comm && comm->p2p;
        if (comm && !p2p && !comm->comm)
            return fail(SAGEICP_ERR_INVALID, "communicator without RCCL needs a connected p2p exchange");
        polled = (!comm || p2p) && env_int("SAGEICP_CHUNKED", 0) == 0;
        max_it = std::min(kMaxIterations, std::max(1, env_int("SAGEICP_MAX_ITER", kMaxIterations)));
        counting = want_stats && g_counting != 0;
        xp.nranks = 1;
        if (!p2p) return SAGEICP_OK;
        xp.nranks = comm->nranks;
        xp.rank = comm->rank;
        for (int r = 0; r < comm->nranks; ++r) xp.block[r] = comm->blocks[r];
        xp.exchanges = comm->d_exchanges.data();
        xp.timeout_ticks = 100000000ull * static_cast<unsigned long long>(std::max(1, env_int("SAGEICP_P2P_TIMEOUT_S", 5)));
        if (const int ticks = env_int("SAGEICP_P2P_TIMEOUT_TICKS", 0))
            xp.timeout_ticks = static_cast<unsigned long long>(ticks);
        return SAGEICP_OK;
    }
    int start_state() const {
        fill_state(sc.h_state.data(), init);
        if (polled) {
            std::memset(sc.h_prog.data(), 0, sizeof(IcpProgress));
            sc.h_state.data()->progress = sc.d_prog;
        }
        HIPCHK(hipMemcpyAsync(sc.d_state.data(), sc.h_state.data(), sizeof(IcpState), hipMemcpyHostToDevice, s));
        return SAGEICP_OK;
    }
    int fetch_state(unsigned nwaves) const {
        if (counting) launch_sum_counters(sc.d_cand.data(), static_cast<int>(nwaves), sc.d_state.data(), s);
        HIPCHK(hipGetLastError());
        HIPCHK(hipMemcpyAsync(sc.h_state.data(), sc.d_state.data(), sizeof(IcpState), hipMemcpyDeviceToHost, s));
        HIPCHK(hipStreamSynchronize(s));
        return SAGEICP_OK;
    }
    int order_frame() const {
        if (n > 0 && n < static_cast<uint64_t>(std::max(0, env_int("SAGEICP_SORT_FROM", kSortFrameFrom))))
            HIPCHK(check_copy_frame(d_frame, sc.d_sorted.data(), static_cast<int>(n), sc.d_state.data(), comm == nullptr, s));
        else if (n > 0)
            HIPCHK(sort_frame(d_frame, sc.d_sorted.data(), static_cast<int>(n), sc.d_state.data(), true, comm == nullptr,
                              m.host.voxel_size, sc.d_keys.data(), sc.d_vals.data(), sc.d_sort_temp.data(),
                              sc.d_sort_temp.capacity(), s));
        return SAGEICP_OK;
    }
};

struct AttemptPlan {
    LoopPlan loop{};
    bool loop_shape = false, use_loop = false, chain = false;
    int lw = 0, chain_grid = 0;
    unsigned loop_waves = 0;
};
static AttemptPlan plan_attempt(const IcpCall &c, const Attempt &a) {
    Scratch &sc = c.sc;
    const sageicp_comm *comm = c.comm;
    const uint64_t n = c.n;
    AttemptPlan p;
    p.loop_shape = (!comm || (c.p2p && !comm->device_shared && env_int("SAGEICP_CHUNKED", 0) == 0)) &&
                   plan_loop(c.m, n, c.sem_th, &p.loop);
    p.lw = p.loop_shape ? p.loop.lw : icp_lw(n, sparse_voxels(c.m));
    p.use_loop = p.loop_shape && !a.no_loop;
    sc.last_fallback = !p.loop_shape ? SAGEICP_LOOP_FALLBACK_DOES_NOT_FIT : (a.no_loop ? SAGEICP_LOOP_FALLBACK_PEER : SAGEICP_LOOP_FALLBACK_NONE);
    if (p.use_loop && sc.loop_cooldown > 0) {
        --sc.loop_cooldown;
        p.use_loop = false;
        sc.last_fallback = SAGEICP_LOOP_FALLBACK_COOLDOWN;
    }
    p.loop_waves = p.use_loop ? static_cast<unsigned>((n + (64u >> p.loop.lw) - 1) / (64u >> p.loop.lw)) : 0u;
    p.chain_grid = n > 0 ? icp_blocks_for(static_cast<int>(n), p.lw) : 0;
    const bool chain_comm = comm && c.p2p && !comm->device_shared && env_int("SAGEICP_CHAIN_COMM", 0) != 0;
    p.chain = !p.loop_shape && (!comm || chain_comm) && c.polled && n > 0 &&
              p.chain_grid / kChainReplicas <= 255 && !a.no_chain && !c.prof2 && env_int("SAGEICP_CHAIN", 1) != 0;
    return p;
}

static bool solver_is_own_launch(const AttemptPlan &p) {
#ifdef SAGE_LOOP_INGRID
    return p.chain;
#else
    return p.chain || p.use_loop;
#endif
}

static LoopParams solver_params(const IcpCall &c, const AttemptPlan &p, double acc_unscale) {
    LoopParams L{};
    L.sh = c.sc.d_loop.data();
    L.st = c.sc.d_state.data();
    L.timeout_ticks = 100000ull * static_cast<unsigned long long>(std::max(1, env_int("SAGEICP_LOOP_TIMEOUT_MS", 50)));
    const int test_ticks = env_int("SAGEICP_LOOP_TIMEOUT_TICKS", 0);
    if (test_ticks) L.timeout_ticks = static_cast<unsigned long long>(test_ticks);
    if (p.chain) {
        L.wgs = p.chain_grid;
        L.copies = kChainReplicas;
        L.progress = c.sc.d_prog;
        L.count_timeout_ticks = std::max<unsigned long long>(L.timeout_ticks, 20ull * 100000ull) * 10ull;
    } else {
        L.nw = p.loop.nw; L.gpw = p.loop.gpw; L.wgs = p.loop.wgs;
        L.copies = kLoopReplicas;
        L.progress = nullptr;
        L.contiguous = env_int("SAGEICP_LOOP_CONTIGUOUS", 0) ? 1 : 0;
        const uint64_t qw = 64u >> p.loop.lw, groups = (c.n + qw - 1) / qw;
        for (int x = 0; x <= 8; ++x) L.xcd_first[x] = static_cast<uint32_t>(groups * x / 8);
        const uint64_t nwg = static_cast<uint64_t>(p.loop.wgs / 8);
        for (int x = 0; x < 8; ++x)
            if (L.contiguous == 1 && (L.xcd_first[x + 1] - L.xcd_first[x] + nwg - 1) / nwg > static_cast<uint64_t>(p.loop.gpw)) L.contiguous = 0;
        L.count_timeout_ticks = L.timeout_ticks;
        L.prio = std::min(3, std::max(0, env_int("SAGEICP_LOOP_PRIO", 3)));
        L.deal = std::min(2, std::max(0, env_int("SAGEICP_LOOP_DEAL", 1)));
    }
    if (c.comm) {
        L.shared_loop = 1;
        if (test_ticks == 0) L.timeout_ticks = std::max(L.timeout_ticks, c.xp.timeout_ticks + 100000000ull);
        if (env_int("SAGEICP_LOOP_COUNT_TIMEOUT_RANK", -1) == c.comm->rank)
            L.count_timeout_ticks = static_cast<unsigned long long>(std::max(1, env_int("SAGEICP_LOOP_COUNT_TIMEOUT_TICKS", 1)));
    }
    L.pose_map = std::min(2, std::max(0, env_int("SAGEICP_LOOP_POSE_MAP", 0)));
    L.max_iterations = c.max_it;
    L.epoch = ++c.sc.loop_epoch;
    for (int i = 0; i < 7; ++i) L.T0[i] = c.init[i];
    L.acc_unscale = acc_unscale;
    return L;
}

struct SolverGuard {
    Scratch &sc;
    unsigned long long epoch = 0;
    bool armed = false;
    explicit SolverGuard(Scratch &s) : sc(s) {}
    ~SolverGuard() {
        if (!armed) return;
        const unsigned long long word = epoch | 0x8000000000000000ull;
        (void)hipMemcpyAsync(&sc.d_loop.data()->go[0], &word, sizeof(word), hipMemcpyHostToDevice, sc.stream.get());
        (void)hipStreamSynchronize(sc.stream.get());
        (void)hipStreamSynchronize(sc.stream2.get());
    }
    int start(const LoopParams &L, const P2pParams &xp) {
        launch_loop_solve(L, xp, sc.stream2.get());
        HIPCHK(hipGetLastError());
        epoch = L.epoch;
        armed = true;
        HIPCHK(hipEventRecord(sc.ev_solve.get(), sc.stream2.get()));
        return SAGEICP_OK;
    }
    void disarm() { armed = false; }
    int send_home_now() {
        sc.go_word = epoch | 0x8000000000000000ull;
        HIPCHK(hipMemcpyAsync(&sc.d_loop.data()->go[0], &sc.go_word, sizeof(sc.go_word), hipMemcpyHostToDevice, sc.stream.get()));
        armed = false;
        return SAGEICP_OK;
    }
};

struct AttemptResult {
    bool looped = false;
    bool chain = false;
    bool chain_gave_up = false;
    int lw = 0;
    bool compact_scan = false;
    double us_nn = 0, us_fin = 0;
    uint32_t nn_launches = 0;
};

static int run_one_launch(const IcpCall &c, const AttemptPlan &p, const IcpParams &ip, const LoopParams &L,
                          SolverGuard &guard, AttemptResult &r) {
    Scratch &sc = c.sc;
    hipStream_t s = c.s;
    int rc;
    if (c.prof && (rc = sc.reserve_events(1))) return rc;
    IcpParams lp = ip;
    lp.filter = p.loop.filter ? ip.filter : 0;
    lp.nwaves = p.loop_waves;
    HIPCHK(hipMemsetAsync(sc.d_loop.data(), 0, offsetof(LoopShared, acc32), s));
    if (c.prof) HIPCHK(hipEventRecord(sc.events[1].get(), s));
    launch_loop(lp, L, p.loop.lw, s);
    if (hipPeekAtLastError() == hipSuccess) guard.disarm();
    if (c.prof) HIPCHK(hipEventRecord(sc.events[2].get(), s));
    if (solver_is_own_launch(p)) HIPCHK(hipStreamWaitEvent(s, sc.ev_solve.get(), 0));
    if ((rc = c.fetch_state(lp.nwaves))) return rc;
    const IcpState &st = *sc.h_state.data();
    r.looped = true;
    if ((st.bad_input && !c.comm) || st.exchange_failed) return SAGEICP_OK;
    if (!st.loop_aborted && st.done) {
        if (c.prof) {
            float a = 0;
            (void)hipEventElapsedTime(&a, sc.events[1].get(), sc.events[2].get());
            r.us_nn = 1e3 * a;
            r.nn_launches = static_cast<uint32_t>(std::max(1, st.iter));
        }
        return SAGEICP_OK;
    }
    r.looped = false;
    if (st.peer_aborted) {
        sc.last_fallback = SAGEICP_LOOP_FALLBACK_PEER;
    } else {
        sc.loop_cooldown = std::max(0, env_int("SAGEICP_LOOP_COOLDOWN", 256));
        if (env_int("SAGEICP_LOOP_TIMEOUT_TICKS", 0) == 0 && env_int("SAGEICP_LOOP_COUNT_TIMEOUT_RANK", -1) < 0 && sc.loop_derate < 16) ++sc.loop_derate;
        ++sc.loop_timeouts;
        sc.last_fallback = SAGEICP_LOOP_FALLBACK_TIMEOUT;
        static std::atomic<int> told{0};
        if (told.exchange(1) == 0 && env_int("SAGEICP_QUIET", 0) == 0)
            std::fprintf(stderr, "sageicp: a wait inside the one-launch ICP loop timed out (the GPU is shared with other work, or "
                                 "fewer workgroups are resident than planned): this frame goes through the launch-per-iteration "
                                 "loop, the next %d calls of this map too, later plans take %d workgroups fewer "
                                 "(sageicp_map_loop_status() reports the state)\n", sc.loop_cooldown, 32 * sc.loop_derate);
    }
    if ((rc = c.start_state())) return rc;
    if (c.counting) HIPCHK(hipMemsetAsync(sc.d_cand.data(), 0, sizeof(unsigned long long) * 2 * (ip.nwaves + 1), s));
    return SAGEICP_OK;
}

struct Iterations {
    const IcpCall &c;
    SolverGuard &guard;
    AttemptResult &r;
    IcpParams &ip;
    const int lw;
    const bool chain;
    Scratch &sc = c.sc;
    hipStream_t s = c.s;
    FinParams fp{};
    unsigned stripes = 0;
    bool lpt = false;
    uint32_t *st_work = nullptr, *st_sorted = nullptr, *st_iota = nullptr, *st_order = nullptr;

    bool sampled(int iteration) const { return c.prof2 || (c.prof && (iteration & 7) == 4); }
    bool measures(int iteration) const { return lpt && (iteration == 0 || iteration == 3 || iteration == 15); }

    int begin(const LoopParams &L) {
        ip.acc = sc.d_acc.data();
        if (chain) {
            HIPCHK(hipMemsetAsync(sc.d_loop.data(), 0, sizeof(LoopShared), s));
            ip.chain = sc.d_loop.data();
            ip.chain_timeout = L.timeout_ticks;
            ip.chain_pose_map = L.pose_map;
            ip.chain_epoch = L.epoch;
            ip.digit_limit = std::min(ip.digit_limit, std::ldexp(1.0, 40));
        }
        fp.st = sc.d_state.data();
        fp.partials = nullptr; fp.nparts = 0; fp.standalone = 0;
        fp.acc = ip.acc;
        fp.acc_unscale = 1.0 / ip.acc_scale;
        fp.mode = c.p2p ? 3 : (c.comm ? 1 : 0);
        if (c.p2p) fp.p2p = c.xp;
        stripes = c.n > 0 ? static_cast<unsigned>(icp_stripes_for(static_cast<int>(c.n), lw)) : 0u;
        lpt = stripes >= 16 && stripes <= sc.sort_cap && stripe_sort_temp_bytes(stripes) <= sc.d_sort_temp.capacity() &&
              env_int("SAGEICP_LPT", c.n >= 40000 ? 1 : 0) != 0;
        st_work = sc.d_keys.data(); st_sorted = sc.d_keys.data() + stripes; st_iota = sc.d_vals.data(); st_order = sc.d_vals.data() + stripes;
        if (lpt) stripe_order_init(st_work, st_iota, stripes, s);
        return SAGEICP_OK;
    }
    int enqueue(int slot, int iteration) {
        const bool ev = sampled(iteration);
        if (ev) HIPCHK(hipEventRecord(sc.events[5 * slot + 1].get(), s));
        ip.stripe_work = measures(iteration) ? st_work : nullptr;
        ip.chain_iter = iteration;
        launch_icp(ip, lw, true, s);
        if (chain && iteration == 0 && hipPeekAtLastError() == hipSuccess) guard.disarm();
        if (measures(iteration)) {
            HIPCHK(stripe_order_sort(st_work, st_sorted, st_iota, st_order, stripes, sc.d_sort_temp.data(), sc.d_sort_temp.capacity(), s));
            ip.stripe_order = st_order;
        }
// ... 28 lines not shown
        int enq = 0;
        unsigned spins = 0;
        unsigned long long idle_word = ~0ull;
        for (;;) {
            const unsigned long long w = *word;
            const int comp = static_cast<int>(w & 0xFFFFFFFFull);
            if (w >> 32) break;
            if (enq < c.max_it && enq - comp < depth) {
                if ((rc = enqueue(enq, enq))) return rc;
                ++enq;
                spins = 0;
                continue;
            }
            __builtin_ia32_pause();
            if ((++spins & 0xFFFFu) == 0) {
                const hipError_t q = hipStreamQuery(s);
                if (q != hipSuccess && q != hipErrorNotReady)
                    return fail(SAGEICP_ERR_HIP, std::string("ICP loop: ") + hipGetErrorString(q));
                if (q == hipSuccess && (*word >> 32) == 0 && enq >= c.max_it)
                    break;
                if (chain && q == hipSuccess) {
                    if (idle_word == *word) break;
                    idle_word = *word;
                } else {
                    idle_word = ~0ull;
                }
            }
        }
        if (chain && guard.armed && (rc = guard.send_home_now())) return rc;
        if (chain) HIPCHK(hipStreamWaitEvent(s, sc.ev_solve.get(), 0));
        if ((rc = c.fetch_state(ip.nwaves))) return rc;
        const IcpState &st = *sc.h_state.data();
        if (chain && (st.loop_aborted || !st.done) && !st.bad_input) {
            static std::atomic<int> told{0};
            if (told.exchange(1) == 0 && env_int("SAGEICP_QUIET", 0) == 0)
                std::fprintf(stderr, "sageicp: a wait inside the chained ICP launches timed out: this frame is registered again with "
                                     "k_fin between the launches\n");
            r.chain_gave_up = true;
            return SAGEICP_OK;
        }
        if (c.prof)
            for (int k = 0; k < st.iter && k < enq; ++k)
                if (sampled(k)) harvest(k);
        return SAGEICP_OK;
    }
    int run_chunked() {
        const IcpState &st = *sc.h_state.data();
        int rc, launched = 0, chunk = 4;
        for (;;) {
            const int todo = std::min(chunk, c.max_it - launched);
            for (int k = 0; k < todo; ++k)
                if ((rc = enqueue(k, launched + k))) return rc;
            if ((rc = c.fetch_state(ip.nwaves))) return rc;
            if (c.prof) {
                const int executed = std::min(todo, st.iter - launched);
                for (int k = 0; k < executed; ++k)
                    if (sampled(launched + k)) harvest(k);
            }
            launched += todo;
            if (st.done || launched >= c.max_it) return SAGEICP_OK;
            chunk = std::min(kChunkMax, chunk * 2);
        }
    }
};

static int run_attempt(const IcpCall &c, const Attempt &a, AttemptResult &r) {
    Scratch &sc = c.sc;
    int rc;
    if ((rc = c.start_state())) return rc;
    const AttemptPlan p = plan_attempt(c, a);
    if ((rc = c.m.dev.ensure_cand(wants_filter(c.m, c.n, c.sem_th), c.s))) return rc;
    if ((rc = sc.reserve_sort(c.n))) return rc;
    IcpParams ip = icp_params(c.m, sc.d_sorted.data(), c.n, c.sem_th, p.lw, a.acc_shift);
    ip.check_done = 1; ip.apply_pose = 1;
    ip.kernel = c.kernel;
    ip.accept_r2 = accept_threshold(c.max_dist);
    ip.counters = c.counting ? sc.d_cand.data() : nullptr;
    if (c.counting) HIPCHK(hipMemsetAsync(sc.d_cand.data(), 0, sizeof(unsigned long long) * 2 * (std::max(ip.nwaves, p.loop_waves) + 1), c.s));
    LoopParams L{};
    SolverGuard guard(sc);
    if (p.use_loop || p.chain) {
        if ((rc = sc.loop_streams())) return rc;
        L = solver_params(c, p, 1.0 / ip.acc_scale);
        if (solver_is_own_launch(p) && (rc = guard.start(L, c.xp))) return rc;
    }
    if ((rc = c.order_frame())) return rc;
    r = AttemptResult{};
    r.lw = p.lw;
    r.chain = p.chain;
    if (p.use_loop && (rc = run_one_launch(c, p, ip, L, guard, r))) return rc;
    r.compact_scan = r.looped ? p.loop.filter && ip.filter : ip.filter != 0;
    if (c.n > 0 && !r.looped) {
        launch_rows(ip, c.s);
        HIPCHK(hipMemsetAsync(sc.d_prev.data(), 0xFF, c.n * sizeof(uint2), c.s));
    }
    HIPCHK(hipMemsetAsync(sc.d_acc.data(), 0, sizeof(long long) * kAccReplicas * kAccWords, c.s));
    if (r.looped) return SAGEICP_OK;
    Iterations it{c, guard, r, ip, p.lw, p.chain};
    if ((rc = it.begin(L))) return rc;
    return c.polled ? it.run_polled() : it.run_chunked();
}

static void fill_stats(sageicp_stats *stats, const IcpState &st, uint64_t n, const AttemptResult &r, double us_upload, double t_begin) {
    std::memset(stats, 0, sizeof(*stats));
    stats->iterations = st.iter; stats->converged = st.converged;
    stats->n_queries = n;
    stats->n_corr_first = st.iter > 0 ? st.n_corr[0] : 0;
    stats->n_corr_last = st.iter > 0 ? st.n_corr[std::min(st.iter, kHistory) - 1] : 0;
    stats->last_step_norm = st.last_step_norm;
    stats->us_upload = us_upload;
    stats->us_nn = r.us_nn; stats->us_fin = r.us_fin;
    stats->nn_launches = r.nn_launches;
    stats->sum_candidates = st.sum_candidates; stats->pairs_evaluated = st.sum_pairs;
    stats->lanes_per_query = 1u << r.lw;
    stats->compact_scan = r.compact_scan ? 1u : 0u;
    stats->single_launch = r.looped ? 1u : 0u;
    for (int i = 0; i < 64 && i < st.iter; ++i) stats->n_corr_hist[i] = st.n_corr[i];
    stats->us_wall = now_us() - t_begin;
}

int run_icp(sageicp_map &m, const Point4 *d_frame, uint64_t n, const double init[7],
            double max_dist, double kernel, double sem_th, sageicp_comm *comm, double out[7],
            sageicp_stats *stats, double us_upload, double t_begin) {
    Scratch &sc = m.sc;
    if (n > kMaxQueries) return fail(SAGEICP_ERR_INVALID, "frame too large (2^26 - 4 points max)");
    int rc;
    IcpCall c{m, d_frame, n, init, max_dist, kernel, sem_th, comm, sc, sc.stream.get(), false, false, false, false, false, 0, P2pParams{}};
    if ((rc = c.constants(stats != nullptr))) return rc;
    if (c.prof && (rc = sc.reserve_events(c.polled ? kMaxIterations : kChunkMax))) return rc;
    Attempt a;
    AttemptResult r;
    const IcpState &st = *sc.h_state.data();
    for (;;) {
        if ((rc = run_attempt(c, a, r))) return rc;
        if (r.chain_gave_up) {
            a.no_chain = true;
        } else if (st.peer_aborted && !r.looped && comm && a.restarts < 4) {
            ++a.restarts;
            a.no_loop = true;
        } else if (st.bad_input) {
            return fail(SAGEICP_ERR_INVALID, "the frame holds a coordinate or label that is not finite (NaN / Inf)");
        } else if (st.acc_overflow && !comm && a.acc_shift < 2) {
            ++a.acc_shift;
        } else {
            break;
        }
    }
    if (st.acc_overflow)
        return fail(SAGEICP_ERR_CAPACITY, "a Gauss-Newton sum left the range of the fixed-point accumulators "
                                          "(coordinates beyond ~10^13 m, a pose guess that is not finite — or, under a communicator, "
                                          "|sum over four queries| >= 2^40: every rank would have to take the same decision)");
    if (st.exchange_failed) {
        if (comm) {
            comm->p2p = false;
            comm->poisoned = true;
        }
        return fail(SAGEICP_ERR_RCCL, "direct exchange: a peer's sums did not arrive in time");
    }
    for (int i = 0; i < 7; ++i) out[i] = st.T[i];
    if (r.looped) ++sc.calls_single_launch; else ++sc.calls_per_iteration;
    if (!r.looped && r.chain) ++sc.calls_chained;
    if (stats) fill_stats(stats, st, n, r, us_upload, t_begin);
    return SAGEICP_OK;
}

int device_update_all(sageicp_map &m, const double *xyzl, uint64_t n, const double pose[7],
                      const Point4 *d_points) {
    if (m.replicas_diverged)
        return fail(SAGEICP_ERR_INVALID, "the copies of this multi-device map diverged in an earlier failed update: Clear() it");
// ... 162 lines not shown
```

### sage-icp_amd/csrc/kernels.h

```cpp
#pragma once

#include <hip/hip_runtime.h>

#include "sageicp_types.h"

namespace sageicp {

constexpr int kRowWords = 32;
constexpr int kRowCq = 27, kRowKey = 28, kRowOcc = 31;
constexpr int kRowLdsStride = 36;

struct LoopShared;
struct IcpParams {
    const Point4 *frame;
    int n;
    const IcpState *st;
    int check_done;
    int apply_pose;
    double voxel_size;
    double inv_voxel_size;
    uint32_t *rows;
    const Slot *table;
    uint32_t mask;
    const Point4 *pts;
    uint32_t pts_bytes;
    int filter;
    int flat;
    const uint4 *cand;
    uint32_t cand_bytes;
    const uint32_t *cand_flags;
    double filt_inv_same;
    double filt_inv_diff;
    double filt_slack;
    double sem_th;
    double dist_init;
    double prune_scale;
    unsigned keep_all;
    int32_t *nn_idx;
    double kernel;
    double accept_r2;
    uint2 *nn_prev;
    uint32_t *work;
    long long *acc;
    double digit_limit;
    double acc_scale;
    uint32_t *stripe_work;
    const uint32_t *stripe_order;
    unsigned long long *counters;
    unsigned nwaves;
#ifdef SAGE_ICP_DELAY_PROBE
    unsigned dbg_delay;
    unsigned dbg_repeat;
#endif
    LoopShared *chain;
    int chain_iter;
    int chain_pose_map;
    unsigned long long chain_timeout;
    unsigned long long chain_epoch;
};

#ifndef SAGE_ICP_WAVES
#define SAGE_ICP_WAVES 4
#endif
constexpr int kIcpWavesPerBlock = SAGE_ICP_WAVES;
int icp_blocks_for(int n, int lw);
size_t icp_lds_bytes(int lw);
void launch_rows(const IcpParams &p, hipStream_t s);
void launch_derive_cand(const Slot *table, uint32_t nslots, const Point4 *pts, uint4 *cand, uint64_t nslots_pts,
                        uint32_t *flags, hipStream_t s);
void launch_icp(const IcpParams &p, int lw, bool fused, hipStream_t s);

struct GnParams {
    const Point4 *src;
    const Point4 *tgt;
    int n;
    double kernel;
    double *partials;
};
int launch_gn(const GnParams &p, hipStream_t s);

constexpr int kAccReplicas = 32;
constexpr int kAccWords = 64;
constexpr int kAccValues = 17;
struct FinParams {
    IcpState *st;
    const double *partials;
    long long *acc;
    double acc_unscale;
    int nparts;
    int mode;
    int standalone;
    P2pParams p2p;
};
void launch_fin(const FinParams &p, hipStream_t s);

#ifndef SAGE_LOOP_REPLICAS
#define SAGE_LOOP_REPLICAS 8
#endif
constexpr int kLoopReplicas = SAGE_LOOP_REPLICAS;
constexpr int kLoopPoseGranules = 25;
constexpr int kLoopPoseCopies = 8;
constexpr int kLoopPoseStride = 32;
constexpr int kChainReplicas = 32;
struct LoopShared {
    long long acc[2][kLoopReplicas][kAccWords];
    unsigned long long pose[kLoopPoseCopies][kLoopPoseStride];
    unsigned long long abort_word[16];
    unsigned long long go[16];
    long long acc32[2][kChainReplicas][kAccWords];
};
struct LoopParams {
    LoopShared *sh;
    IcpState *st;
    int nw;
    int gpw;
    int wgs;
    int contiguous;
    uint32_t xcd_first[9];
    unsigned long long timeout_ticks;
    unsigned long long count_timeout_ticks;
    int max_iterations;
    unsigned long long epoch;
    double T0[7];
    double acc_unscale;
    int shared_loop;
    int prio;
    int deal;
    int copies;
    int pose_map;
    IcpProgress *progress;
};
struct LoopArgs {
    IcpParams P;
    LoopParams L;
    double face_slack;
};
#ifndef SAGE_LOOP_OCC
#define SAGE_LOOP_OCC 7
#endif
constexpr int kLoopMaxWavesHost = 8;
constexpr int kLoopStripeHost = 4;
constexpr int kLoopStateWords = 24;
size_t loop_lds_bytes(int lw, int nw, int gpw);
int loop_blocks_per_cu(int lw, bool filter, int nw, size_t lds);
void launch_loop(const IcpParams &p, const LoopParams &l, int lw, hipStream_t s);
void launch_loop_solve(const LoopParams &l, const P2pParams &x, hipStream_t s);

constexpr int kMaxPartials = 1 << 16;
constexpr uint64_t kMaxQueries = (1ull << 26) - 4;

void launch_tf(Point4 *pts, int n, const IcpState *st, hipStream_t s);
void launch_scatter_points(const uint32_t *idx, const Point4 *vals, uint32_t n, Point4 *pts,
                           hipStream_t s);
void launch_scatter_slots(const uint32_t *idx, const Slot *vals, uint32_t n, Slot *table,
                          hipStream_t s);
void launch_scatter_u32(const uint32_t *idx, const uint32_t *vals, uint32_t n, uint32_t *dst, hipStream_t s);
void launch_sum_counters(const unsigned long long *c, int n, IcpState *st, hipStream_t s);

struct VdsParams {
    const Point4 *in;
    int n;
    int do_crop;
    double max_range, min_range, label_max_range;
    int n_groups;
    const int *group_counts;
    const int *group_labels;
    double group_vs[8];
    double scale;
    unsigned long long *keys;
    uint32_t *winner;
    uint32_t mask;
    Point4 *tmp;
    uint32_t *slot_of;
    uint32_t *sort_key;
    uint32_t *sort_val;
    int *overflow;
    unsigned long long *out_keys;
};
size_t vds_sort_temp_bytes(int n);
void launch_vds_permute(const Point4 *in, const uint32_t *perm, uint32_t n, Point4 *out, hipStream_t s);
hipError_t voxel_downsample_device(const VdsParams &P, void *sort_temp, size_t sort_temp_bytes,
                                   uint32_t *d_n_kept, Point4 *out, hipStream_t s);

struct DeskewTangent {
    double v[6];
};
void launch_deskew(const Point4 *in, Point4 *out, const double *ts, int n, const DeskewTangent &d, hipStream_t s);

constexpr int kIngestBadTimestamp = 8;
struct IngestArgs {
    const unsigned char *xyz;
    const unsigned char *label;
    unsigned long long xyz_stride, label_stride;
    int xyz_dtype, label_dtype;
    int n;
    const double *ts;
    double *ts_out;
    int *flags;
};
void launch_ingest(const IngestArgs &a, Point4 *out, hipStream_t s);

constexpr int kOccNonFinite = 16;
constexpr int kOccMaxSide = 4096;
struct OccGrid {
    double lo[3], hi[3];
    double x_res, y_res;
    int h, w;
};
struct OccTransform {
    double R[9];
    double t[3];
};
struct OccDecision {
    unsigned long long key;
    unsigned long long inter;
    int take;
    int pad;
};
inline uint32_t occ_words(const OccGrid &g) { return static_cast<uint32_t>((static_cast<uint64_t>(g.h) * g.w + 31) / 32); }
void launch_occ_keep(const Point4 *in, Point4 *out, int n, int *flags, hipStream_t s);
void launch_occ_draw(const Point4 *in, int n, const OccGrid &g, const OccTransform *tf, uint32_t *id, uint32_t *cur,
                     int *flags, bool force_global, hipStream_t s);
void launch_occ_decide(uint32_t *key, const uint32_t *cand, const uint32_t *cur, uint32_t words, int force, double th,
                       OccDecision *out, hipStream_t s);
void launch_occ_unpack(const uint32_t *bits, const OccGrid &g, unsigned char *out, hipStream_t s);

size_t sort_temp_bytes(int n);
size_t stripe_sort_temp_bytes(unsigned stripes);
void stripe_order_init(uint32_t *work, uint32_t *iota, unsigned stripes, hipStream_t s);
hipError_t stripe_order_sort(uint32_t *work, uint32_t *work_sorted, const uint32_t *iota, uint32_t *order, unsigned stripes,
                             void *temp, size_t temp_bytes, hipStream_t s);
int icp_stripes_for(int n, int lw);
hipError_t sort_frame(const Point4 *d_in, Point4 *d_out, int n, IcpState *st, bool apply_pose, bool stop_on_bad,
                      double voxel_size, uint32_t *keys, uint32_t *vals, void *temp,
                      size_t temp_bytes, hipStream_t s);
constexpr int kSortFrameFrom = 16384;
hipError_t check_copy_frame(const Point4 *d_in, Point4 *d_out, int n, IcpState *st, bool stop_on_bad, hipStream_t s);

}
```

### sage-icp_amd/csrc/kernels.hip

```cpp

#include <hip/hip_runtime.h>

#include <algorithm>
#include <cfloat>
#include <cstdlib>
#include <type_traits>
#include <vector>

#ifndef SAGE_ICP_STRIPE
#define SAGE_ICP_STRIPE 8
#endif
#ifndef SAGE_ICP_OCC
#define SAGE_ICP_OCC 6
#endif

#include "kernels.h"
#include "se3_math.h"
#include "sageicp_types.h"
#include "probes.h"

namespace sageicp {


template <int CTRL>
// ... 571 lines not shown
}
size_t icp_lds_bytes(int lw) {
    return sizeof(uint32_t) * (kWgHeaderWords + kIcpWavesPerBlock * icp_wave_words(lw));
}

void launch_rows(const IcpParams &p, hipStream_t s) {
    if (p.n <= 0) return;
    hipLaunchKernelGGL(k_rows, dim3((p.n + 7) / 8), dim3(256), 0, s, p);
}

template <int LW>
static void launch_icp_lw(const IcpParams &p, bool fused, hipStream_t s) {
    const int grid = icp_blocks_for(p.n, LW);
    const size_t lds = icp_lds_bytes(LW);
    const dim3 g(grid), b(64 * kIcpWavesPerBlock);
    constexpr bool kBoth = LW == 1 || LW == 2;
    const bool flat = LW >= 3 || (kBoth && p.flat);
    auto go = [&](auto flat_c) {
        constexpr bool F = decltype(flat_c)::value;
        if (p.filter) {
            if (fused) hipLaunchKernelGGL((k_icp<LW, true, true, F>), g, b, lds, s, p);
            else hipLaunchKernelGGL((k_icp<LW, false, true, F>), g, b, lds, s, p);
        } else {
            if (fused) hipLaunchKernelGGL((k_icp<LW, true, false, F>), g, b, lds, s, p);
            else hipLaunchKernelGGL((k_icp<LW, false, false, F>), g, b, lds, s, p);
        }
    };
    if constexpr (kBoth) {
        if (flat) go(std::true_type{});
        else go(std::false_type{});
    } else if constexpr (LW >= 3) {
        go(std::true_type{});
    } else {
        go(std::false_type{});
    }
}
void launch_icp(const IcpParams &p, int lw, bool fused, hipStream_t s) {
    if (p.n <= 0) return;
    switch (lw) {
        case 0: launch_icp_lw<0>(p, fused, s); break;
        case 1: launch_icp_lw<1>(p, fused, s); break;
        case 2: launch_icp_lw<2>(p, fused, s); break;
        case 3: launch_icp_lw<3>(p, fused, s); break;
        default: launch_icp_lw<4>(p, fused, s); break;
    }
}

size_t loop_lds_bytes(int lw, int nw, int gpw) {
    return sizeof(uint32_t) * LoopLds<size_t>(lw, static_cast<size_t>(nw), static_cast<size_t>(gpw)).end;
}
static const void *loop_kernel(int lw, bool filter) {
#define SAGE_LOOP_K(LW_, F_) reinterpret_cast<const void *>(&k_loop<LW_, F_>)
    switch (lw) {
        case 1: return filter ? SAGE_LOOP_K(1, true) : SAGE_LOOP_K(1, false);
        case 2: return filter ? SAGE_LOOP_K(2, true) : SAGE_LOOP_K(2, false);
        case 3: return filter ? SAGE_LOOP_K(3, true) : SAGE_LOOP_K(3, false);
        case 4: return filter ? SAGE_LOOP_K(4, true) : SAGE_LOOP_K(4, false);
        default: return nullptr;
    }
#undef SAGE_LOOP_K
}
int loop_blocks_per_cu(int lw, bool filter, int nw, size_t lds) {
    if (nw < 1 || nw > kLoopMaxWaves || lds > 160 * 1024) return 0;
    const void *k = loop_kernel(lw, filter);
    if (!k) return 0;
    if (lds > 64 * 1024 && hipFuncSetAttribute(k, hipFuncAttributeMaxDynamicSharedMemorySize, 160 * 1024) != hipSuccess) return 0;
    int nb = 0;
    if (hipOccupancyMaxActiveBlocksPerMultiprocessor(&nb, k, 64 * nw, lds) != hipSuccess) return 0;
    return nb;
}
void launch_loop(const IcpParams &p, const LoopParams &l, int lw, hipStream_t s) {
    const size_t lds = loop_lds_bytes(lw, l.nw, l.gpw);
    LoopArgs a;
    a.P = p;
    a.L = l;
    a.face_slack = 1e-9 * p.voxel_size;
    void *args[] = {&a};
#ifdef SAGE_LOOP_INGRID
    (void)hipLaunchKernel(loop_kernel(lw, p.filter != 0), dim3(l.wgs + 1), dim3(64 * l.nw), args, lds, s);
#else
    (void)hipLaunchKernel(loop_kernel(lw, p.filter != 0), dim3(l.wgs), dim3(64 * l.nw), args, lds, s);
#endif
}
void launch_loop_solve(const LoopParams &l, const P2pParams &x, hipStream_t s) {
    SolveArgs a;
    a.L = l;
    a.X = x;
    if (l.copies == kChainReplicas) hipLaunchKernelGGL(k_loop_solve<kChainReplicas>, dim3(1), dim3(64), 0, s, a);
    else hipLaunchKernelGGL(k_loop_solve<kLoopReplicas>, dim3(1), dim3(64), 0, s, a);
}

int launch_gn(const GnParams &p, hipStream_t s) {
    long blocks = (static_cast<long>(p.n) + 255) / 256;
    if (blocks > 128) blocks = 128;
    if (blocks < 1) blocks = 1;
    hipLaunchKernelGGL(k_gn, dim3(static_cast<int>(blocks)), dim3(256), 0, s, p);
    return static_cast<int>(blocks);
}

void launch_fin(const FinParams &p, hipStream_t s) {
    hipLaunchKernelGGL(k_fin, dim3(1), dim3(kFinThreads), 0, s, p);
}

void launch_tf(Point4 *pts, int n, const IcpState *st, hipStream_t s) {
    if (n <= 0) return;
    hipLaunchKernelGGL(k_tf, dim3((n + 255) / 256), dim3(256), 0, s, pts, n, st);
}

}
```

### sage-icp_amd/csrc/loop_kernel.h

```cpp
#pragma once

#include "loop_deal.h"

namespace sageicp {


__device__ __forceinline__ int exchange_sums_wave(double *S, const P2pParams &X, unsigned long long g) {
    const int lane = static_cast<int>(threadIdx.x & 63u);
    const int slot = static_cast<int>(g & 1ull);
    const unsigned long long tag = g + 1ull;
    if (lane < kNumSums) {
        const double v = S[lane];
        for (int r = 0; r < X.nranks; ++r)
            __hip_atomic_store(&X.block[r]->sums[slot][X.rank][lane], v, __ATOMIC_RELAXED, __HIP_MEMORY_SCOPE_SYSTEM);
    }
    asm volatile("s_waitcnt vmcnt(0)" ::: "memory");
    __builtin_amdgcn_fence(__ATOMIC_RELEASE, "");
    asm volatile("s_waitcnt vmcnt(0)" ::: "memory");
    if (lane == 0)
        for (int r = 0; r < X.nranks; ++r)
            __hip_atomic_store(&X.block[r]->flag[X.rank], tag, __ATOMIC_RELAXED, __HIP_MEMORY_SCOPE_SYSTEM);
    P2pBlock *mine = X.block[X.rank];
    bool late = false, gone = false;
    if (lane < X.nranks) {
        const unsigned long long t0 = __builtin_amdgcn_s_memrealtime();
        while (__hip_atomic_load(&mine->flag[lane], __ATOMIC_RELAXED, __HIP_MEMORY_SCOPE_SYSTEM) < tag) {
            __builtin_amdgcn_s_sleep(2);
            if (__builtin_amdgcn_s_memrealtime() - t0 > X.timeout_ticks) {
                late = true;
                break;
            }
        }
        __builtin_amdgcn_fence(__ATOMIC_ACQUIRE, "");
        gone = __hip_atomic_load(&mine->abort_tag[lane], __ATOMIC_RELAXED, __HIP_MEMORY_SCOPE_SYSTEM) == tag;
    }
    late = __any(late);
    gone = __any(gone);
    __builtin_amdgcn_fence(__ATOMIC_ACQUIRE, "");
    if (lane < kNumSums) {
        double s = 0.0;
        for (int r = 0; r < X.nranks; ++r)
            s += __hip_atomic_load(&mine->sums[slot][r][lane], __ATOMIC_RELAXED, __HIP_MEMORY_SCOPE_SYSTEM);
        S[lane] = s;
    }
    __builtin_amdgcn_wave_barrier();
    return gone ? 2 : (late ? 1 : 0);
}
__device__ __forceinline__ void exchange_abort_wave(const P2pParams &X, unsigned long long g) {
    const int lane = static_cast<int>(threadIdx.x & 63u);
    if (lane == 0)
        for (int r = 0; r < X.nranks; ++r)
            __hip_atomic_store(&X.block[r]->abort_tag[X.rank], g + 1ull, __ATOMIC_RELAXED, __HIP_MEMORY_SCOPE_SYSTEM);
    asm volatile("s_waitcnt vmcnt(0)" ::: "memory");
    __builtin_amdgcn_fence(__ATOMIC_RELEASE, "");
    asm volatile("s_waitcnt vmcnt(0)" ::: "memory");
    if (lane == 0)
        for (int r = 0; r < X.nranks; ++r)
            __hip_atomic_store(&X.block[r]->flag[X.rank], g + 1ull, __ATOMIC_RELAXED, __HIP_MEMORY_SCOPE_SYSTEM);
    asm volatile("s_waitcnt vmcnt(0)" ::: "memory");
}

struct SolveLds {
    double T[14];
    double S[kNumSums];
};
__device__ __forceinline__ unsigned long long readlane_u64(unsigned long long v, int src) {
    const unsigned lo = static_cast<unsigned>(__builtin_amdgcn_readlane(static_cast<int>(static_cast<unsigned>(v)), src));
    const unsigned hi = static_cast<unsigned>(__builtin_amdgcn_readlane(static_cast<int>(static_cast<unsigned>(v >> 32)), src));
    return (static_cast<unsigned long long>(hi) << 32) | lo;
}
__device__ __forceinline__ void loop_give_up(const LoopParams &L, LoopShared *sh, IcpState *st, int it, unsigned long long tag, int lane,
                                             bool peer) {
    if (lane == 0) {
        st_agent(&sh->abort_word[0], 1ull);
        st->loop_aborted = 1;
        if (peer) st->peer_aborted = 1;
        if (L.progress)
            __hip_atomic_store(&L.progress->word, (1ull << 32) | static_cast<unsigned long long>(it), __ATOMIC_RELAXED,
                               __HIP_MEMORY_SCOPE_SYSTEM);
    }
    if (const int al = lane_now(); al < kLoopPoseCopies) st_agent(&sh->pose[al][24], (tag << 32) | 2ull);
}
template <int COPIES>
__device__ __forceinline__ unsigned loop_finish_iteration(const LoopParams &L, const P2pParams &X, SolveLds &m, int it,
                                                          unsigned long long &xg) {
    LoopShared *sh = L.sh;
    IcpState *st = L.st;
    const int lane = static_cast<int>(threadIdx.x & 63u);
    double *sT = m.T, *S = m.S;
    const unsigned long long tag = static_cast<unsigned long long>(it) + 1ull;

    double sum = 0.0;
    bool overflow;
    {
        const long long per = static_cast<long long>(L.wgs / COPIES);
        long long (*acc)[kAccWords] = COPIES == kLoopReplicas ? sh->acc[it & 1] : sh->acc32[it & 1];
        long long v[COPIES];
        const unsigned long long t0 = __builtin_amdgcn_s_memrealtime();
        for (;;) {
#pragma unroll
            for (int r = 0; r < COPIES; ++r)
                v[r] = __hip_atomic_load(&acc[r][lane], __ATOMIC_RELAXED, __HIP_MEMORY_SCOPE_AGENT);
            bool ok = true;
            if (lane <= 3 * kAccValues) {
#pragma unroll
                for (int r = 0; r < COPIES; ++r) ok &= (v[r] & 255ll) == per;
            }
            if (__all(ok)) break;
            unsigned long long ab = 0ull;
            if (lane == 0) ab = ld_agent(&sh->abort_word[0]);
            const bool late = __builtin_amdgcn_s_memrealtime() - t0 > L.count_timeout_ticks;
            if (__any(ab != 0ull) || late) {
                loop_give_up(L, sh, st, it, tag, lane, false);
                if (X.nranks > 1) {
                    exchange_abort_wave(X, xg);
                    xg += 1ull;
                    if (lane == 0) *X.exchanges = xg;
                }
                return 2u;
            }
            __builtin_amdgcn_s_sleep(1);
        }
        LOOP_STAMP_SOLVER(it, 0);
        long long d = 0;
        if (lane <= 3 * kAccValues) {
#pragma unroll
            for (int r = 0; r < COPIES; ++r) d += (v[r] - per) >> 8;
        }
#pragma unroll
        for (int r = 0; r < COPIES; ++r)
            __hip_atomic_store(&acc[r][lane], 0ll, __ATOMIC_RELAXED, __HIP_MEMORY_SCOPE_AGENT);
        const int sl = lane_now();
        const int s3 = 3 * (sl < kAccValues ? sl : 0);
        const double a = static_cast<double>(__shfl(d, s3));
        const double b = static_cast<double>(__shfl(d, s3 + 1));
        const double c = static_cast<double>(__shfl(d, s3 + 2));
        if (lane < kAccValues) {
            sum = a + (b * 9.094947017729282e-13 + c * 8.271806125530277e-25);
            if (lane < kCount) sum *= L.acc_unscale;
        }
        if (lane < kNumSums) S[lane] = sum;
        overflow = readlane_u64(static_cast<unsigned long long>(d), 3 * kAccValues) != 0ull;
        __builtin_amdgcn_wave_barrier();
    }
    LOOP_STAMP_SOLVER(it, 1);

    bool exchange_failed = false;
    if (X.nranks > 1) {
        const int ex = exchange_sums_wave(S, X, xg);
        xg += 1ull;
        if (lane == 0) *X.exchanges = xg;
        exchange_failed = ex == 1;
        if (ex == 2) {
            loop_give_up(L, sh, st, it, tag, lane, true);
            return 2u;
        }
    }

    double x[6], est[7], nrm;
    solve_normal_equations_t<WaveLanes>(S, x);
    LOOP_STAMP_SOLVER2(it, 0);
    se3_exp_sqrt_t<WaveLanes>(x, est, SAGE_SQNORM6(x), nrm);
    LOOP_STAMP_SOLVER2(it, 1);
    double rhs[7], Tn[7];
    {
        const double *src = sT + (lane == 1 ? 7 : 0);
#pragma unroll
        for (int i = 0; i < 7; ++i) rhs[i] = src[i];
    }
    se3_mul(est, rhs, Tn);
    __builtin_amdgcn_wave_barrier();
    if (lane < 2) {
        double *dst = sT + (lane == 1 ? 7 : 0);
#pragma unroll
        for (int i = 0; i < 7; ++i) dst[i] = Tn[i];
    }
    double Rn[9];
    quat_to_mat(Tn, Rn);
    LOOP_STAMP_SOLVER2(it, 2);
    if (!(x[3] * x[3] + x[4] * x[4] + x[5] * x[5] < 9.0) || fabs(nrm - kEstimationThreshold) < 1e-12) {
        double lg[6];
        se3_log(est, lg);
        nrm = sqrt(SAGE_SQNORM6(lg));
    }
    LOOP_STAMP_SOLVER2(it, 3);
    const bool converged = nrm < kEstimationThreshold;
    unsigned done = (converged || it + 1 >= L.max_iterations) ? 1u : 0u;
    if (overflow && !L.shared_loop) done = 1u;
    if (exchange_failed) done = 1u;
    const int pl = lane_now();
    const int gl = (pl & 31) - 2;
    uint32_t word = done;
#pragma unroll
    for (int i = 0; i < 12; ++i) {
        const unsigned long long v = static_cast<unsigned long long>(__double_as_longlong(i < 9 ? Rn[i] : Tn[i - 5]));
        if ((gl >> 1) == i) word = static_cast<uint32_t>((gl & 1) ? v >> 32 : v);
    }
    LOOP_STAMP_SOLVER(it, 2);
    asm volatile("s_waitcnt vmcnt(0)" ::: "memory");
    if (gl >= 0 && gl < kLoopPoseGranules) {
#pragma unroll
        for (int c = 0; c < kLoopPoseCopies; c += 2)
            st_agent(&sh->pose[c + (pl >> 5)][gl], (tag << 32) | word);
    }
    if (lane == 0) {
        if (it < kHistory) st->n_corr[it] = static_cast<uint32_t>(S[kCount]);
        if (overflow) st->acc_overflow = 1;
        if (exchange_failed) st->exchange_failed = 1;
        if (done) {
#pragma unroll
            for (int i = 0; i < 7; ++i) st->T[i] = Tn[i];
#pragma unroll
            for (int i = 0; i < 9; ++i) st->R[i] = Rn[i];
            st->last_step_norm = nrm;
            st->iter = it + 1;
            st->done = 1;
            st->converged = (converged && !exchange_failed) ? 1 : 0;
        }
    }
    if (done && lane == 1) {
#pragma unroll
        for (int i = 0; i < 7; ++i) st->T_icp[i] = Tn[i];
    }
    if (L.progress && lane == 0)
        __hip_atomic_store(&L.progress->word, (static_cast<unsigned long long>(done ? 1u : 0u) << 32) | static_cast<unsigned long long>(it + 1),
                           __ATOMIC_RELAXED, __HIP_MEMORY_SCOPE_SYSTEM);
    if (done && lane < kNumSums) st->sums[lane] = S[lane];
    LOOP_STAMP_SOLVER(it, 3);
    return done;
}

struct SolveArgs {
    LoopParams L;
    P2pParams X;
};
template <int COPIES>
__global__ __launch_bounds__(64) void k_loop_solve(SolveArgs A) {
    __shared__ SolveLds m;
    __builtin_amdgcn_s_setprio(3);
    {
        const int lane = static_cast<int>(threadIdx.x & 63u);
        const unsigned long long t0 = __builtin_amdgcn_s_memrealtime();
        for (;;) {
            const unsigned long long g = ld_agent(&A.L.sh->go[0]);
            if ((g & 0x7FFFFFFFFFFFFFFFull) == A.L.epoch) {
                if (g >> 63) return;
                break;
            }
            if (__builtin_amdgcn_s_memrealtime() - t0 > 1000ull * A.L.timeout_ticks + 1000000000ull) {
                if (lane == 0) A.L.st->loop_aborted = 1;
                return;
            }
            __builtin_amdgcn_s_sleep(32);
        }
        if (lane < 14) m.T[lane] = lane < 7 ? A.L.T0[lane] : (lane == 10 ? 1.0 : 0.0);
    }
    unsigned long long xg = A.X.nranks > 1 ? *A.X.exchanges : 0ull;
    __builtin_amdgcn_wave_barrier();
    for (int it = 0;; ++it) {
        auto ka = __builtin_amdgcn_kernarg_segment_ptr();
        asm volatile("" : "+s"(ka));
        const SolveArgs &K = *(const SolveArgs *)(ka);
        if (loop_finish_iteration<COPIES>(K.L, K.X, m, it, xg)) return;
    }
}

#ifndef SAGE_LOOP_POLL_SLEEP
#define SAGE_LOOP_POLL_SLEEP 8
#endif

__device__ __forceinline__ void loop_set_priority(unsigned gi, int nw, int prio) {
    const unsigned rk = gi >= static_cast<unsigned>(nw) ? static_cast<unsigned>(prio) : 3u - min(gi, 3u);
    switch (rk) {
        case 0: __builtin_amdgcn_s_setprio(0); break;
        case 1: __builtin_amdgcn_s_setprio(1); break;
        case 2: __builtin_amdgcn_s_setprio(2); break;
        default: __builtin_amdgcn_s_setprio(3); break;
    }
}

template <int LW, bool FILT>
__global__ __launch_bounds__(64 * kLoopMaxWaves) __attribute__((amdgpu_waves_per_eu(SAGE_LOOP_OCC, 8)))
void k_loop(LoopArgs A) {
    extern __shared__ __attribute__((aligned(16))) uint32_t smem[];
    constexpr int QW = 64 >> LW;
    const IcpParams &P = A.P;
    const LoopParams &L = A.L;
    const int wv = __builtin_amdgcn_readfirstlane(static_cast<int>(threadIdx.x >> 6));
    const int nw = L.nw;
    const unsigned gpw = static_cast<unsigned>(L.gpw);
    double *s_pose = reinterpret_cast<double *>(smem + kLpPose);

    {
        const bool bad = !L.shared_loop && P.st->bad_input;
        if (blockIdx.x == 0 && threadIdx.x == 0)
            st_agent(&L.sh->go[0], L.epoch | (bad ? 0x8000000000000000ull : 0ull));
        if (bad) return;
    }

#ifdef SAGE_LOOP_INGRID
    if (blockIdx.x == gridDim.x - 1u) {
        if (threadIdx.x >= 64u) return;
        SolveLds &m = *reinterpret_cast<SolveLds *>(smem);
        const int lane = static_cast<int>(threadIdx.x & 63u);
        if (lane < 14) m.T[lane] = lane < 7 ? L.T0[lane] : (lane == 10 ? 1.0 : 0.0);
        __builtin_amdgcn_wave_barrier();
        P2pParams X{};
        X.nranks = 1;
        unsigned long long xg = 0ull;
        for (int it = 0;; ++it)
            if (loop_finish_iteration<kLoopReplicas>(L, X, m, it, xg)) return;
    }
#endif

    unsigned g0, gcnt;
    {
        const unsigned xcd = blockIdx.x & 7u, jb = blockIdx.x >> 3;
        const unsigned ngroups = (static_cast<unsigned>(P.n) + QW - 1u) / QW;
        unsigned lo = 0u, cnt = ngroups, idx, nwg;
        if (L.contiguous == 1) {
            lo = L.xcd_first[xcd];
            cnt = L.xcd_first[xcd + 1u] - lo;
            idx = jb;
            nwg = static_cast<unsigned>(L.wgs) >> 3;
        } else {
            idx = ((jb / kLoopStripe) * 8u + xcd) * kLoopStripe + (jb % kLoopStripe);
            nwg = static_cast<unsigned>(L.wgs);
        }
        const unsigned base = cnt / nwg, extra = cnt - base * nwg;
        g0 = lo + idx * base + min(idx, extra);
        gcnt = min(gpw, base + (idx < extra ? 1u : 0u));
    }
    constexpr unsigned BPW = QW / 4;
    const unsigned nblk_max = gpw * BPW;
    const LoopLds<unsigned> lds0(LW, static_cast<unsigned>(nw), gpw);
    uint32_t *perm0 = smem + lds0.perm;
    uint32_t *work0 = smem + lds0.work;
    uint32_t *state0 = smem + lds0.state;

    if (threadIdx.x < 9) s_pose[threadIdx.x] = P.st->R[threadIdx.x];
    else if (threadIdx.x < 12) s_pose[threadIdx.x] = P.st->T[4 + threadIdx.x - 9];
    if (threadIdx.x == 0) {
        smem[kLpArrive] = 0u;
        smem[kLpNext] = 0u;
        smem[kLpDone] = 0u;
        smem[kLpIter] = 0u;
        PROBE_LOOP_CLEAR_STATS(smem);
    }
    if (L.deal && (threadIdx.x & 63u) == 0u) {
        unsigned hw;
        asm volatile("s_getreg_b32 %0, hwreg(HW_REG_HW_ID)" : "=s"(hw));
        const unsigned simd = (hw >> 4) & 3u, slot = hw & 15u;
        smem[kLpFirst + static_cast<unsigned>(wv)] = L.deal == 2 ? loopdeal::formula(simd, slot, static_cast<unsigned>(nw))
                                                                 : loopdeal::loop_deal_unit(simd, slot, static_cast<unsigned>(nw));
    }
    for (unsigned i = threadIdx.x; i < 2u * kWgAccWords; i += blockDim.x) smem[kLpAcc + i] = 0u;
    for (unsigned i = threadIdx.x; i < nblk_max; i += blockDim.x) {
        perm0[i] = i;
        work0[i] = 0u;
    }
    for (unsigned sl = threadIdx.x; sl < gcnt * QW; sl += blockDim.x) {
        const unsigned q = g0 * QW + sl;
        const Point4 f = P.frame[q < static_cast<unsigned>(P.n) ? q : 0u];
        {
            uint32_t *lst = state0 + sl * kLoopStateWords;
            *reinterpret_cast<Point4 *>(lst) = f;
            Point4 z;
            z.x = z.y = z.z = z.l = 0.0;
            *reinterpret_cast<Point4 *>(lst + 8) = z;
            *reinterpret_cast<uint4 *>(lst + kStPrev) = make_uint4(0xFFFFFFFFu, 0u, static_cast<uint32_t>(kNoVoxel),
                                                                   static_cast<uint32_t>(kNoVoxel));
            *reinterpret_cast<uint4 *>(lst + kStPrev + 4) = make_uint4(static_cast<uint32_t>(kNoVoxel), 0u, 0u, 0u);
        }
    }
    __syncthreads();
    if (L.deal) {
        unsigned claimed = 0u, kept = 0u, table[kLoopMaxWaves];
        for (int w2 = 0; w2 < nw; ++w2) {
            const unsigned pr = smem[kLpFirst + static_cast<unsigned>(w2)];
            table[w2] = pr;
            if (!((claimed >> pr) & 1u)) { claimed |= 1u << pr; kept |= 1u << w2; }
        }
        for (int w2 = 0; w2 < nw; ++w2)
            if (!((kept >> w2) & 1u)) {
                const unsigned pr = static_cast<unsigned>(__builtin_ctz(~claimed));
                table[w2] = pr;
                claimed |= 1u << pr;
            }
        __syncthreads();
        if (threadIdx.x == 0) {
            for (int w2 = 0; w2 < nw; ++w2) smem[kLpFirst + static_cast<unsigned>(w2)] = table[w2];
            smem[kLpNext] = static_cast<unsigned>(nw);
        }
        __syncthreads();
// ... 157 lines not shown
```

### sage-icp_amd/csrc/sageicp_types.h

```cpp
#pragma once

#include <cstdint>

#if defined(__HIPCC__)
#include <hip/hip_runtime.h>
#define SAGE_HD __host__ __device__
#else
#define SAGE_HD
#endif

#ifndef SAGE_SQNORM3_ORDER
#define SAGE_SQNORM3_ORDER 2
#endif
#define SAGE_SQNORM3_A(xx, yy, zz) ((xx) + ((yy) + (zz)))
#define SAGE_SQNORM3_B(xx, yy, zz) (((xx) + (yy)) + (zz))
#if SAGE_SQNORM3_ORDER == 0
#define SAGE_SQNORM3_NN SAGE_SQNORM3_A
#define SAGE_SQNORM3_RESID SAGE_SQNORM3_A
#define SAGE_SQNORM3_FAR SAGE_SQNORM3_A
#define SAGE_SQNORM3_ACCEPT SAGE_SQNORM3_A
#define SAGE_SQNORM3_CROP SAGE_SQNORM3_A
#elif SAGE_SQNORM3_ORDER == 1
#define SAGE_SQNORM3_NN SAGE_SQNORM3_B
#define SAGE_SQNORM3_RESID SAGE_SQNORM3_B
#define SAGE_SQNORM3_FAR SAGE_SQNORM3_B
#define SAGE_SQNORM3_ACCEPT SAGE_SQNORM3_B
#define SAGE_SQNORM3_CROP SAGE_SQNORM3_B
#else
#define SAGE_SQNORM3_NN SAGE_SQNORM3_B
#define SAGE_SQNORM3_RESID SAGE_SQNORM3_B
#define SAGE_SQNORM3_FAR SAGE_SQNORM3_B
#define SAGE_SQNORM3_ACCEPT SAGE_SQNORM3_B
#define SAGE_SQNORM3_CROP SAGE_SQNORM3_B
#endif
#if SAGE_SQNORM3_ORDER == 2
#define SAGE_SQNORM6(a) ((((a)[0] * (a)[0]) + (((a)[2] * (a)[2]) + ((a)[4] * (a)[4]))) + \
                         (((a)[1] * (a)[1]) + (((a)[3] * (a)[3]) + ((a)[5] * (a)[5]))))
#else
#define SAGE_SQNORM6(a) ((((((a)[0] * (a)[0] + (a)[1] * (a)[1]) + (a)[2] * (a)[2]) + (a)[3] * (a)[3]) + \
                          (a)[4] * (a)[4]) + (a)[5] * (a)[5])
#endif

namespace sageicp {

struct alignas(16) Slot {
    int32_t x, y, z;
    uint32_t blk;
};
constexpr uint32_t kEmptySlot = 0xFFFFFFFFu;
constexpr uint32_t kTombstone = 0xFFFFFFFEu;
constexpr int32_t kTombKey = 0x7F7F7F7F;
constexpr uint32_t kNoSlot = 0xFFFFFFFFu;
constexpr int kMaxBlockBits = 24;
constexpr int kMaxCap = 255;
constexpr uint32_t kUnitPoints = 4;
constexpr uint32_t kMaxUnits = (1u << 24) - 2;
constexpr int kMaxClasses = 4;
constexpr uint32_t kNoRegion = 0xFFFFFFFFu;

SAGE_HD inline uint32_t voxel_hash(int32_t x, int32_t y, int32_t z) {
    uint32_t h = static_cast<uint32_t>(x) * 0x9E3779B1u;
    h ^= static_cast<uint32_t>(y) * 0x85EBCA77u + (h << 6) + (h >> 2);
    h ^= static_cast<uint32_t>(z) * 0xC2B2AE3Du + (h << 6) + (h >> 2);
    h ^= h >> 16;
    h *= 0x7FEB352Du;
    h ^= h >> 15;
    h *= 0x846CA68Bu;
    h ^= h >> 16;
    return h;
}

struct alignas(32) Point4 {
    double x, y, z, l;
};

constexpr int kMaxIterations = 500;
constexpr double kEstimationThreshold = 1e-4;
constexpr int kNumSums = 20;
constexpr int kHistory = 512;

struct IcpProgress {
    unsigned long long word;
    unsigned long long pad_[7];
};

constexpr int kMaxRanks = 8;
struct P2pBlock {
    unsigned long long flag[kMaxRanks];
    double sums[2][kMaxRanks][kNumSums];
    unsigned long long abort_tag[kMaxRanks];
};
struct P2pParams {
    int nranks, rank;
    P2pBlock *block[kMaxRanks];
    unsigned long long *exchanges;
    unsigned long long timeout_ticks;
};

struct IcpState {
    double T[7];
    double R[9];
    double T_icp[7];
    double last_step_norm;
    int32_t iter;
    int32_t done;
    int32_t converged;
    int32_t peer_aborted;
    double sums[kNumSums];
    unsigned long long sum_candidates;
    unsigned long long sum_pairs;
    uint32_t n_corr[kHistory];
    IcpProgress *progress;
    int32_t exchange_failed;
    int32_t acc_overflow;
    int32_t loop_aborted;
    int32_t bad_input;
};

enum Sum : int {
    kW = 0,
    kWsx, kWsy, kWsz,
    kWxx, kWxy, kWxz, kWyy, kWyz, kWzz,
    kWrx, kWry, kWrz,
    kWcx, kWcy, kWcz,
    kCount,
};

}
```

### sage-icp_amd/csrc/sort.hip

```cpp
#include <hip/hip_runtime.h>
#include <cstring>

#include <rocprim/rocprim.hpp>

#include "kernels.h"

namespace sageicp {

__device__ __forceinline__ uint32_t spread10(uint32_t v) {
    v &= 1023u;
    v = (v | (v << 16)) & 0x030000FFu;
    v = (v | (v << 8)) & 0x0300F00Fu;
    v = (v | (v << 4)) & 0x030C30C3u;
    v = (v | (v << 2)) & 0x09249249u;
    return v;
}

template <bool APPLY_POSE>
__global__ __launch_bounds__(256) void k_morton_keys(const Point4 *pts, int n, IcpState *st, int stop_on_bad,
                                                     double voxel_size, uint32_t *keys,
                                                     uint32_t *vals) {
    const int i = blockIdx.x * 256 + threadIdx.x;
    if (i >= n) return;
    const Point4 f = pts[i];
    if (!(fabs(f.x) <= 1.7976931348623157e308 && fabs(f.y) <= 1.7976931348623157e308 &&
          fabs(f.z) <= 1.7976931348623157e308 && fabs(f.l) <= 1.7976931348623157e308)) {
        st->bad_input = 1;
        if (stop_on_bad) {
            st->done = 1;
            if (IcpProgress *pg = st->progress)
                __hip_atomic_store(&pg->word, 1ull << 32, __ATOMIC_RELAXED, __HIP_MEMORY_SCOPE_SYSTEM);
        }
    }
    double x = f.x, y = f.y, z = f.z;
    if (APPLY_POSE) {
        const double *R = st->R;
        const double *T = st->T;
        x = R[0] * f.x + R[1] * f.y + R[2] * f.z + T[4];
        y = R[3] * f.x + R[4] * f.y + R[5] * f.z + T[5];
        z = R[6] * f.x + R[7] * f.y + R[8] * f.z + T[6];
    }
    const int cx = static_cast<int>(x / voxel_size) + 512;
    const int cy = static_cast<int>(y / voxel_size) + 512;
    const int cz = static_cast<int>(z / voxel_size) + 512;
    keys[i] = spread10(static_cast<uint32_t>(cx)) | (spread10(static_cast<uint32_t>(cy)) << 1) |
              (spread10(static_cast<uint32_t>(cz)) << 2);
    vals[i] = static_cast<uint32_t>(i);
}

__global__ __launch_bounds__(256) void k_gather(const Point4 *in, const uint32_t *perm, int n,
                                                Point4 *out) {
    const int i = blockIdx.x * 256 + threadIdx.x;
    if (i >= n) return;
    out[i] = in[perm[i]];
}

__global__ __launch_bounds__(256) void k_check_copy(const Point4 *pts, int n, IcpState *st, int stop_on_bad, Point4 *out) {
    const int i = blockIdx.x * 256 + threadIdx.x;
    if (i >= n) return;
    const Point4 f = pts[i];
    if (!(fabs(f.x) <= 1.7976931348623157e308 && fabs(f.y) <= 1.7976931348623157e308 &&
          fabs(f.z) <= 1.7976931348623157e308 && fabs(f.l) <= 1.7976931348623157e308)) {
        st->bad_input = 1;
        if (stop_on_bad) {
            st->done = 1;
            if (IcpProgress *pg = st->progress)
                __hip_atomic_store(&pg->word, 1ull << 32, __ATOMIC_RELAXED, __HIP_MEMORY_SCOPE_SYSTEM);
        }
    }
    out[i] = f;
}
hipError_t check_copy_frame(const Point4 *d_in, Point4 *d_out, int n, IcpState *st, bool stop_on_bad, hipStream_t s) {
    if (n <= 0) return hipSuccess;
    hipLaunchKernelGGL(k_check_copy, dim3((n + 255) / 256), dim3(256), 0, s, d_in, n, st, stop_on_bad ? 1 : 0, d_out);
    return hipGetLastError();
}

size_t sort_temp_bytes(int n) {
    size_t bytes = 0;
    uint32_t *k = nullptr;
    (void)rocprim::radix_sort_pairs(nullptr, bytes, k, k, k, k, static_cast<unsigned>(n), 0, 30);
    return bytes;
}

hipError_t sort_frame(const Point4 *d_in, Point4 *d_out, int n, IcpState *st, bool apply_pose, bool stop_on_bad,
                      double voxel_size, uint32_t *keys, uint32_t *vals, void *temp,
                      size_t temp_bytes, hipStream_t s) {
    if (n <= 0) return hipSuccess;
    const int grid = (n + 255) / 256;
    if (apply_pose)
        hipLaunchKernelGGL(k_morton_keys<true>, dim3(grid), dim3(256), 0, s, d_in, n, st, stop_on_bad ? 1 : 0,
                           voxel_size, keys, vals);
    else
        hipLaunchKernelGGL(k_morton_keys<false>, dim3(grid), dim3(256), 0, s, d_in, n, st, stop_on_bad ? 1 : 0,
                           voxel_size, keys, vals);
    hipError_t e = rocprim::radix_sort_pairs(temp, temp_bytes, keys, keys + n, vals, vals + n,
                                             static_cast<unsigned>(n), 0, 30, s);
    if (e != hipSuccess) return e;
    hipLaunchKernelGGL(k_gather, dim3(grid), dim3(256), 0, s, d_in, vals + n, n, d_out);
    return hipGetLastError();
}

__global__ __launch_bounds__(256) void k_stripe_init(uint32_t *work, uint32_t *iota, unsigned n) {
    const unsigned i = blockIdx.x * 256u + threadIdx.x;
    if (i >= n) return;
    work[i] = 0u;
    iota[i] = i;
}
size_t stripe_sort_temp_bytes(unsigned stripes) {
    size_t bytes = 0;
    uint32_t *k = nullptr;
    (void)rocprim::radix_sort_pairs_desc(nullptr, bytes, k, k, k, k, stripes, 0, 32);
    return bytes;
}
void stripe_order_init(uint32_t *work, uint32_t *iota, unsigned stripes, hipStream_t s) {
    if (stripes) hipLaunchKernelGGL(k_stripe_init, dim3((stripes + 255u) / 256u), dim3(256), 0, s, work, iota, stripes);
}
hipError_t stripe_order_sort(uint32_t *work, uint32_t *work_sorted, const uint32_t *iota, uint32_t *order, unsigned stripes,
                             void *temp, size_t temp_bytes, hipStream_t s) {
    if (!stripes) return hipSuccess;
    hipError_t e = rocprim::radix_sort_pairs_desc(temp, temp_bytes, work, work_sorted, iota, order, stripes, 0, 32, s);
    if (e != hipSuccess) return e;
    return hipMemsetAsync(work, 0, sizeof(uint32_t) * stripes, s);
}

}
```

Before: 253.2.

## Replace rocprim frame sort with custom radix passes and mirror ICP state to host

After: 254.4 (median of 5 runs). No clear change (+0.5%).

```diff
diff --git a/include/sageicp.h b/include/sageicp.h
--- a/include/sageicp.h
+++ b/include/sageicp.h
@@ -246,6 +246,10 @@
                                        const sageicp_device_points *tgt_out ,
                                        int64_t *query_idx_out , uint64_t idx_cap,
                                        void *stream , uint64_t *n_out);
+
+int sageicp_frame_order(int device, const double *rows, uint64_t n, const double guess[7], double voxel_size,
+                        uint32_t *perm_out);
+int sageicp_frame_order_path(uint64_t n);
 
 typedef struct sageicp_quality {
     double fitness, rmse, step_norm;
diff --git a/profiles/call_timeline.py b/profiles/call_timeline.py
--- /dev/null
+++ b/profiles/call_timeline.py
@@ -0,0 +1,81 @@
+import collections
+import csv
+import glob
+import os
+import sys
+
+
+def _rows(d, suffix):
+    out = []
+    for path in glob.glob(os.path.join(d, "**", "*" + suffix), recursive=True):
+        with open(path, newline="") as fh:
+            out += list(csv.DictReader(fh))
+    return out
+
+
+def short(name):
+    name = name.split("(")[0]
+    for lead in ("void ", "sageicp::", "rocprim::detail::", "rocprim::"):
+        name = name.replace(lead, "")
+    return name if len(name) <= 56 else name[:53] + "..."
+
+
+def load(d):
+    ops = []
+    for r in _rows(d, "kernel_trace.csv"):
+        ops.append((int(r["Start_Timestamp"]), int(r["End_Timestamp"]), short(r["Kernel_Name"])))
+    for r in _rows(d, "memory_copy_trace.csv"):
+        ops.append((int(r["Start_Timestamp"]), int(r["End_Timestamp"]), "copy " + r.get("Direction", "?").replace("MEMORY_COPY_", "")))
+    ops.sort()
+    return ops
+
+
+def main():
+    d = sys.argv[1]
+    calls = int(sys.argv[2]) if len(sys.argv) > 2 else 5
+    ops = load(d)
+    loops = [i for i, o in enumerate(ops) if o[2].startswith("k_loop<")]
+    counted = [any(o[2].startswith("k_sum_counters") for o in ops[a:b]) for a, b in zip(loops, loops[1:] + [len(ops)])]
+    timed = [li for li, c in zip(loops, counted) if not c]
+    if len(timed) != calls:
+        sys.exit("%d launches of k_loop without counters in %s, %d expected" % (len(timed), d, calls))
+    if len(sys.argv) > 3:
+        print("wall time of a call (ms_per_step): %s ms" % sys.argv[3])
+    print("k_loop: %.1f us (mean of the %d timed calls)" % (sum(ops[li][1] - ops[li][0] for li in timed) / 1e3 / calls, calls))
+    per_op = collections.defaultdict(list)
+    outside, spans = [], []
+    for c, li in enumerate(timed[1:], start=1):
+        prev = timed[c - 1]
+        t0 = ops[prev][1]
+        window = [o for o in ops[prev + 1:li] if o[0] >= t0 or o[2].startswith("k_loop_solve")]
+        print("\ncall %d: k_loop %.1f us; %.1f us from the end of the k_loop before it to its start"
+              % (c + 1, (ops[li][1] - ops[li][0]) / 1e3, (ops[li][0] - t0) / 1e3))
+        print("  %10s %9s %9s  %s" % ("start", "duration", "gap", "operation"))
+        last = t0
+        seen = collections.Counter()
+        for s, e, name in window:
+            solve = name.startswith("k_loop_solve")
+            print("  %10.1f %9.1f %9s  %s" % ((s - t0) / 1e3, (e - s) / 1e3, "" if solve else "%.1f" % ((s - last) / 1e3),
+                                               name + (" (second stream, resident to the end of the call)" if solve else "")))
+            if solve:
+                continue
+            seen[name] += 1
+            per_op["%s #%d" % (name, seen[name])].append(((e - s) / 1e3, (s - last) / 1e3))
+            last = max(last, e)
+        print("  %10.1f %9s %9.1f  k_loop starts" % ((ops[li][0] - t0) / 1e3, "", (ops[li][0] - last) / 1e3))
+        outside.append((ops[li][0] - t0) / 1e3)
+        keyk = [o for o in window if o[2].startswith("k_morton_keys") or o[2].startswith("k_frame_")]
+        gath = [o for o in window if o[2].startswith("k_gather") or o[2].startswith("k_frame_")]
+        if keyk and gath:
+            spans.append((gath[-1][1] - keyk[0][0]) / 1e3)
+    print("\nmeans over the %d windows between the timed calls: %.1f us between two k_loop [%.1f-%.1f]%s"
+          % (len(outside), sum(outside) / len(outside), min(outside), max(outside),
+             "; the frame's order, first key kernel to the end of the gather: %.1f us" % (sum(spans) / len(spans)) if spans else ""))
+    print("  %9s %9s  %s" % ("duration", "gap", "operation (in the order of the last call)"))
+    for name, v in per_op.items():
+        print("  %9.1f %9.1f  %s%s" % (sum(x[0] for x in v) / len(v), sum(x[1] for x in v) / len(v), name,
+                                       "" if len(v) == len(outside) else "  (%d of %d windows)" % (len(v), len(outside))))
+
+
+if __name__ == "__main__":
+    main()
diff --git a/sage-icp_amd/__init__.py b/sage-icp_amd/__init__.py
--- a/sage-icp_amd/__init__.py
+++ b/sage-icp_amd/__init__.py
@@ -298,6 +298,8 @@
     ("sageicp_get_correspondences_device", C.c_int,
      [C.c_void_p, C.POINTER(DeviceFrame), _dp, C.c_double, C.c_double, C.POINTER(DevicePoints), C.POINTER(DevicePoints),
       C.c_void_p, C.c_uint64, C.c_void_p, _u64p]),
+    ("sageicp_frame_order", C.c_int, [C.c_int, _dp, C.c_uint64, _dp, C.c_double, C.c_void_p]),
+    ("sageicp_frame_order_path", C.c_int, [C.c_uint64]),
     ("sageicp_registration_quality", C.c_int,
      [C.c_void_p, _dp, C.c_uint64, _dp, C.c_double, C.c_double, C.c_double, C.POINTER(Quality)]),
     ("sageicp_registration_quality_device", C.c_int,
@@ -1120,6 +1122,21 @@
     return out
 
 
+def frame_order(rows, guess, voxel_size, device=0):
+    pts, fp = _d(rows)
+    g, gp = _d(guess)
+    if g.size != 7:
+        raise ValueError("a pose is (qx, qy, qz, qw, tx, ty, tz)")
+    n = pts.reshape(-1, 4).shape[0]
+    out = np.zeros(n, dtype=np.uint32)
+    _check(lib().sageicp_frame_order(device, fp, n, gp, float(voxel_size), out.ctypes.data_as(C.c_void_p)))
+    return out
+
+
+def frame_order_path(n):
+    return int(lib().sageicp_frame_order_path(int(n)))
+
+
 def occupancy_grid(frame, bounds=KEY_FRAME_BOUNDS, occ_size=KEY_FRAME_OCC_SIZE, pose=None, device=0, labels=None):
     params = occupancy_params(bounds, occ_size, 0.0)
     out = np.zeros((params.occ_h, params.occ_w), dtype=np.uint8)
diff --git a/sage-icp_amd/build.py b/sage-icp_amd/build.py
--- a/sage-icp_amd/build.py
+++ b/sage-icp_amd/build.py
@@ -9,7 +9,7 @@
            "csrc/map_device.hip", "csrc/capi_run.hip", "csrc/prep.hip", "csrc/capi.hip", "csrc/capi_pipeline.hip",
            "csrc/capi_outputs.hip", "csrc/caller_mem.hip", "csrc/correspond.hip", "csrc/quality.hip", "csrc/score.hip",
            "csrc/capi_query.hip", "csrc/capi_relocalize.hip", "csrc/archive.hip", "csrc/capi_archive.hip"]
-HEADERS = ["csrc/kernels.h", "csrc/dev_buffer.h", "csrc/sageicp_types.h", "csrc/se3_math.h", "csrc/host_map.hpp", "csrc/pipeline.hpp", "csrc/map_update.h", "csrc/egress.h", "csrc/msg.h", "csrc/metrics.hpp", "csrc/robin_order.hpp", "csrc/capi_internal.h", "csrc/prep.h", "csrc/prefetch.h", "csrc/dyn_rules.h", "csrc/probes.h", "csrc/icp_body.h", "csrc/row_shift.h", "csrc/fin_kernel.h", "csrc/loop_kernel.h", "csrc/loop_deal.h", "csrc/caller_mem.h", "csrc/outputs.h", "csrc/map_device.h", "csrc/replay_pool.h", "csrc/correspond.h", "csrc/quality.h", "csrc/score.h", "csrc/accept.h", "csrc/archive.h", "csrc/query.h",
+HEADERS = ["csrc/kernels.h", "csrc/dev_buffer.h", "csrc/sageicp_types.h", "csrc/se3_math.h", "csrc/host_map.hpp", "csrc/pipeline.hpp", "csrc/map_update.h", "csrc/egress.h", "csrc/msg.h", "csrc/metrics.hpp", "csrc/robin_order.hpp", "csrc/capi_internal.h", "csrc/prep.h", "csrc/prefetch.h", "csrc/dyn_rules.h", "csrc/probes.h", "csrc/icp_body.h", "csrc/row_shift.h", "csrc/fin_kernel.h", "csrc/loop_kernel.h", "csrc/loop_deal.h", "csrc/frame_sort.h", "csrc/caller_mem.h", "csrc/outputs.h", "csrc/map_device.h", "csrc/replay_pool.h", "csrc/correspond.h", "csrc/quality.h", "csrc/score.h", "csrc/accept.h", "csrc/archive.h", "csrc/query.h",
            "../include/sageicp.h"]
 OUT = os.path.join(HERE, "libsageicp_hip.so")
 OBJ_DIR = os.path.join(HERE, "build")
diff --git a/sage-icp_amd/csrc/capi_internal.h b/sage-icp_amd/csrc/capi_internal.h
--- a/sage-icp_amd/csrc/capi_internal.h
+++ b/sage-icp_amd/csrc/capi_internal.h
@@ -145,7 +145,8 @@
     int last_fallback = 0;
     DevBuf<unsigned long long> d_cand;
     DevBuf<IcpState> d_state;
-    PinnedBuf<IcpState> h_state;
+    PinnedBuf<IcpState, hipHostMallocMapped | hipHostMallocCoherent> h_state;
+    IcpState *d_hstate = nullptr;
     PinnedBuf<IcpProgress, hipHostMallocMapped | hipHostMallocCoherent> h_prog;
     IcpProgress *d_prog = nullptr;
     std::vector<OwnedEvent> events;
@@ -210,6 +211,7 @@
         HIPCHK(h_state.reserve(1));
         HIPCHK(h_prog.reserve(1));
         HIPCHK(hipHostGetDevicePointer(reinterpret_cast<void **>(&d_prog), h_prog.data(), 0));
+        HIPCHK(hipHostGetDevicePointer(reinterpret_cast<void **>(&d_hstate), h_state.data(), 0));
         return SAGEICP_OK;
     }
     int loop_streams() {
@@ -385,6 +387,8 @@
 void fill_state(IcpState *st, const double init[7]);
 double accept_threshold(double max_dist);
 bool sparse_voxels(const sageicp_map &m);
+bool frame_is_sorted(uint64_t n);
+int sort_impl();
 bool wants_filter(const sageicp_map &m, uint64_t n, double sem_th);
 IcpParams icp_params(const sageicp_map &m, const Point4 *d_queries, uint64_t n, double sem_th, int lw, int acc_shift);
 int run_icp(sageicp_map &m, const Point4 *d_frame, uint64_t n, const double init[7], double max_dist, double kernel,
diff --git a/sage-icp_amd/csrc/capi_query.hip b/sage-icp_amd/csrc/capi_query.hip
--- a/sage-icp_amd/csrc/capi_query.hip
+++ b/sage-icp_amd/csrc/capi_query.hip
@@ -33,7 +33,7 @@
 int QueryCall::sort_and_search(const Point4 *d_rows, uint64_t n, double sem_th, bool read_verdict) {
     HIPCHK(sort_frame(d_rows, sc.d_sorted.data(), static_cast<int>(n), sc.d_state.data(), false, false,
                       m.host.voxel_size, sc.d_keys.data(), sc.d_vals.data(), sc.d_sort_temp.data(),
-                      sc.d_sort_temp.capacity(), stream()));
+                      sc.d_sort_temp.capacity(), sort_impl(), ZeroWords{nullptr, 0u}, stream()));
     if (read_verdict) {
         HIPCHK(hipMemcpyAsync(sc.h_state.data(), sc.d_state.data(), sizeof(IcpState), hipMemcpyDeviceToHost, stream()));
         if (int rc = wait()) return rc;
@@ -295,6 +295,46 @@
     return SAGEICP_OK;
 }
 
+int sageicp_frame_order(int device, const double *rows, uint64_t n, const double guess[7], double voxel_size, uint32_t *perm_out) {
+    if (!guess || (n && (!rows || !perm_out))) return fail(SAGEICP_ERR_INVALID, "null argument");
+    if (!(voxel_size > 0.0)) return fail(SAGEICP_ERR_INVALID, "voxel_size must be positive");
+    if (n > kMaxQueries) return fail(SAGEICP_ERR_INVALID, "too many rows (2^26 - 4 max)");
+    if (!all_finite(rows, n)) return refuse_non_finite("FrameOrder", "frame");
+    if (n == 0) return SAGEICP_OK;
+    if (!frame_is_sorted(n)) {
+        for (uint64_t i = 0; i < n; ++i) perm_out[i] = static_cast<uint32_t>(i);
+        return SAGEICP_OK;
+    }
+    if (int rc = require_device(device)) return rc;
+    HIPCHK(hipSetDevice(device));
+    DevBuf<Point4> d_in, d_out;
+    DevBuf<uint32_t> d_keys, d_vals;
+    DevBuf<unsigned char> d_temp;
+    DevBuf<IcpState> d_state;
+    OwnedStream stream;
+    HIPCHK(d_in.reserve(n));
+    HIPCHK(d_out.reserve(n));
+    HIPCHK(d_keys.reserve(2 * n));
+    HIPCHK(d_vals.reserve(2 * n));
+    HIPCHK(d_temp.reserve(sort_temp_bytes(static_cast<int>(n))));
+    HIPCHK(d_state.reserve(1));
+    HIPCHK(stream.create());
+    IcpState st;
+    fill_state(&st, guess);
+    HIPCHK(hipMemcpyAsync(d_state.data(), &st, sizeof(IcpState), hipMemcpyHostToDevice, stream.get()));
+    HIPCHK(hipMemcpyAsync(d_in.data(), rows, n * sizeof(Point4), hipMemcpyHostToDevice, stream.get()));
+    HIPCHK(sort_frame(d_in.data(), d_out.data(), static_cast<int>(n), d_state.data(), true, false, voxel_size, d_keys.data(),
+                      d_vals.data(), d_temp.data(), d_temp.capacity(), sort_impl(), ZeroWords{nullptr, 0u}, stream.get()));
+    HIPCHK(hipMemcpyAsync(perm_out, d_vals.data() + n, n * sizeof(uint32_t), hipMemcpyDeviceToHost, stream.get()));
+    HIPCHK(hipStreamSynchronize(stream.get()));
+    return SAGEICP_OK;
+}
+
+int sageicp_frame_order_path(uint64_t n) {
+    if (n == 0 || !frame_is_sorted(n)) return 0;
+    return n <= kMaxQueries && frame_sort_own_path(sort_impl(), static_cast<long long>(n)) ? 2 : 1;
+}
+
 int sageicp_get_correspondences_device(const sageicp_map *map, const sageicp_device_frame *frame, const double pose[7],
                                        double max_dist, double sem_th, const sageicp_device_points *src_out,
                                        const sageicp_device_points *tgt_out, int64_t *query_idx_out, uint64_t idx_cap,
diff --git a/sage-icp_amd/csrc/capi_run.hip b/sage-icp_amd/csrc/capi_run.hip
--- a/sage-icp_amd/csrc/capi_run.hip
+++ b/sage-icp_amd/csrc/capi_run.hip
@@ -222,6 +222,11 @@
     return ok;
 }
 
+bool frame_is_sorted(uint64_t n) {
+    return n >= static_cast<uint64_t>(std::max(0, env_int("SAGEICP_SORT_FROM", kSortFrameFrom)));
+}
+int sort_impl() { return env_int("SAGEICP_SORT_IMPL", 1) != 0 ? 1 : 0; }
+
 struct Attempt {
     int acc_shift = 0;
     int restarts = 0;
@@ -278,13 +283,33 @@
         HIPCHK(hipStreamSynchronize(s));
         return SAGEICP_OK;
     }
-    int order_frame() const {
-        if (n > 0 && n < static_cast<uint64_t>(std::max(0, env_int("SAGEICP_SORT_FROM", kSortFrameFrom))))
-            HIPCHK(check_copy_frame(d_frame, sc.d_sorted.data(), static_cast<int>(n), sc.d_state.data(), comm == nullptr, s));
+    int await_state(unsigned long long epoch, unsigned nwaves, hipEvent_t done) const {
+        HIPCHK(hipGetLastError());
+        const volatile unsigned long long *word = &sc.h_prog.data()->final_epoch;
+        for (unsigned spins = 1;; ++spins) {
+            if (*word == epoch) break;
+            __builtin_ia32_pause();
+            if ((spins & 0xFFu) == 0) {
+                const hipError_t q = hipStreamQuery(s);
+                if (q == hipSuccess && *word != epoch) return fetch_state(nwaves);
+                if (q != hipSuccess && q != hipErrorNotReady) return fail(SAGEICP_ERR_HIP, std::string("ICP loop: ") + hipGetErrorString(q));
+            }
+        }
+        std::atomic_thread_fence(std::memory_order_acquire);
+        if (done) {
+            hipError_t q;
+            while ((q = hipEventQuery(done)) == hipErrorNotReady) __builtin_ia32_pause();
+            if (q != hipSuccess) return fail(SAGEICP_ERR_HIP, std::string("ICP loop: ") + hipGetErrorString(q));
+        }
+        return SAGEICP_OK;
+    }
+    int order_frame(ZeroWords zero) const {
+        if (n > 0 && !frame_is_sorted(n))
+            HIPCHK(check_copy_frame(d_frame, sc.d_sorted.data(), static_cast<int>(n), sc.d_state.data(), comm == nullptr, zero, s));
         else if (n > 0)
             HIPCHK(sort_frame(d_frame, sc.d_sorted.data(), static_cast<int>(n), sc.d_state.data(), true, comm == nullptr,
                               m.host.voxel_size, sc.d_keys.data(), sc.d_vals.data(), sc.d_sort_temp.data(),
-                              sc.d_sort_temp.capacity(), s));
+                              sc.d_sort_temp.capacity(), sort_impl(), zero, s));
         return SAGEICP_OK;
     }
 };
@@ -294,6 +319,7 @@
     bool loop_shape = false, use_loop = false, chain = false;
     int lw = 0, chain_grid = 0;
     unsigned loop_waves = 0;
+    bool zero_in_kernel = false, mirror = false;
 };
 static AttemptPlan plan_attempt(const IcpCall &c, const Attempt &a) {
     Scratch &sc = c.sc;
@@ -311,6 +337,10 @@
         sc.last_fallback = SAGEICP_LOOP_FALLBACK_COOLDOWN;
     }
     p.loop_waves = p.use_loop ? static_cast<unsigned>((n + (64u >> p.loop.lw) - 1) / (64u >> p.loop.lw)) : 0u;
+    p.zero_in_kernel = p.use_loop && env_int("SAGEICP_ZERO_IN_KERNEL", 1) != 0;
+#ifndef SAGE_LOOP_INGRID
+    p.mirror = p.use_loop && !comm && c.polled && !c.counting && env_int("SAGEICP_STATE_MIRROR", 1) != 0;
+#endif
     p.chain_grid = n > 0 ? icp_blocks_for(static_cast<int>(n), p.lw) : 0;
     const bool chain_comm = comm && c.p2p && !comm->device_shared && env_int("SAGEICP_CHAIN_COMM", 0) != 0;
     p.chain = !p.loop_shape && (!comm || chain_comm) && c.polled && n > 0 &&
@@ -378,8 +408,8 @@
         (void)hipStreamSynchronize(sc.stream.get());
         (void)hipStreamSynchronize(sc.stream2.get());
     }
-    int start(const LoopParams &L, const P2pParams &xp) {
-        launch_loop_solve(L, xp, sc.stream2.get());
+    int start(const LoopParams &L, const P2pParams &xp, const StateMirror &mirror) {
+        launch_loop_solve(L, xp, mirror, sc.stream2.get());
         HIPCHK(hipGetLastError());
         epoch = L.epoch;
         armed = true;
@@ -414,13 +444,13 @@
     IcpParams lp = ip;
     lp.filter = p.loop.filter ? ip.filter : 0;
     lp.nwaves = p.loop_waves;
-    HIPCHK(hipMemsetAsync(sc.d_loop.data(), 0, offsetof(LoopShared, acc32), s));
+    if (!p.zero_in_kernel) HIPCHK(hipMemsetAsync(sc.d_loop.data(), 0, offsetof(LoopShared, acc32), s));
     if (c.prof) HIPCHK(hipEventRecord(sc.events[1].get(), s));
     launch_loop(lp, L, p.loop.lw, s);
     if (hipPeekAtLastError() == hipSuccess) guard.disarm();
     if (c.prof) HIPCHK(hipEventRecord(sc.events[2].get(), s));
     if (solver_is_own_launch(p)) HIPCHK(hipStreamWaitEvent(s, sc.ev_solve.get(), 0));
-    if ((rc = c.fetch_state(lp.nwaves))) return rc;
+    if ((rc = p.mirror ? c.await_state(L.epoch, lp.nwaves, c.prof ? sc.events[2].get() : nullptr) : c.fetch_state(lp.nwaves))) return rc;
     const IcpState &st = *sc.h_state.data();
     r.looped = true;
     if ((st.bad_input && !c.comm) || st.exchange_failed) return SAGEICP_OK;
@@ -615,9 +645,13 @@
     if (p.use_loop || p.chain) {
         if ((rc = sc.loop_streams())) return rc;
         L = solver_params(c, p, 1.0 / ip.acc_scale);
-        if (solver_is_own_launch(p) && (rc = guard.start(L, c.xp))) return rc;
-    }
-    if ((rc = c.order_frame())) return rc;
+        const StateMirror mirror = p.mirror ? StateMirror{sc.d_hstate, &sc.d_prog->final_epoch} : StateMirror{nullptr, nullptr};
+        if (solver_is_own_launch(p) && (rc = guard.start(L, c.xp, mirror))) return rc;
+    }
+    const ZeroWords zero = p.zero_in_kernel ? ZeroWords{reinterpret_cast<unsigned long long *>(sc.d_loop.data()),
+                                                        static_cast<unsigned>(offsetof(LoopShared, acc32) / sizeof(unsigned long long))}
+                                            : ZeroWords{nullptr, 0u};
+    if ((rc = c.order_frame(zero))) return rc;
     r = AttemptResult{};
     r.lw = p.lw;
     r.chain = p.chain;
diff --git a/sage-icp_amd/csrc/frame_sort.h b/sage-icp_amd/csrc/frame_sort.h
--- /dev/null
+++ b/sage-icp_amd/csrc/frame_sort.h
@@ -0,0 +1,24 @@
+#pragma once
+
+#include <cstddef>
+#include <cstdint>
+
+namespace sageicp {
+
+constexpr int kFrameSortTile = 2048;
+constexpr int kFrameSortMaxTiles = 128;
+constexpr int kFrameSortPasses = 4;
+constexpr int kFrameSortDigits = 256;
+
+inline bool frame_sort_own_path(int impl, long long n) {
+    return impl != 0 && n > 0 && n <= static_cast<long long>(kFrameSortTile) * kFrameSortMaxTiles;
+}
+inline size_t frame_sort_tiles(long long n) {
+    return n > 0 ? static_cast<size_t>((n + kFrameSortTile - 1) / kFrameSortTile) : 0u;
+}
+inline size_t frame_sort_own_bytes(long long n) {
+    const size_t tiles = frame_sort_tiles(n) < static_cast<size_t>(kFrameSortMaxTiles) ? frame_sort_tiles(n) : static_cast<size_t>(kFrameSortMaxTiles);
+    return sizeof(uint32_t) * kFrameSortPasses * tiles * kFrameSortDigits;
+}
+
+}
diff --git a/sage-icp_amd/csrc/kernels.h b/sage-icp_amd/csrc/kernels.h
--- a/sage-icp_amd/csrc/kernels.h
+++ b/sage-icp_amd/csrc/kernels.h
@@ -3,6 +3,7 @@
 #include <hip/hip_runtime.h>
 
 #include "sageicp_types.h"
+#include "frame_sort.h"
 
 namespace sageicp {
 
@@ -144,7 +145,11 @@
 size_t loop_lds_bytes(int lw, int nw, int gpw);
 int loop_blocks_per_cu(int lw, bool filter, int nw, size_t lds);
 void launch_loop(const IcpParams &p, const LoopParams &l, int lw, hipStream_t s);
-void launch_loop_solve(const LoopParams &l, const P2pParams &x, hipStream_t s);
+struct StateMirror {
+    IcpState *st;
+    unsigned long long *epoch_word;
+};
+void launch_loop_solve(const LoopParams &l, const P2pParams &x, const StateMirror &m, hipStream_t s);
 
 constexpr int kMaxPartials = 1 << 16;
 constexpr uint64_t kMaxQueries = (1ull << 26) - 4;
@@ -226,6 +231,10 @@
 void launch_occ_unpack(const uint32_t *bits, const OccGrid &g, unsigned char *out, hipStream_t s);
 
 size_t sort_temp_bytes(int n);
+struct ZeroWords {
+    unsigned long long *words;
+    unsigned n;
+};
 size_t stripe_sort_temp_bytes(unsigned stripes);
 void stripe_order_init(uint32_t *work, uint32_t *iota, unsigned stripes, hipStream_t s);
 hipError_t stripe_order_sort(uint32_t *work, uint32_t *work_sorted, const uint32_t *iota, uint32_t *order, unsigned stripes,
@@ -233,8 +242,8 @@
 int icp_stripes_for(int n, int lw);
 hipError_t sort_frame(const Point4 *d_in, Point4 *d_out, int n, IcpState *st, bool apply_pose, bool stop_on_bad,
                       double voxel_size, uint32_t *keys, uint32_t *vals, void *temp,
-                      size_t temp_bytes, hipStream_t s);
+                      size_t temp_bytes, int impl, ZeroWords zero, hipStream_t s);
 constexpr int kSortFrameFrom = 16384;
-hipError_t check_copy_frame(const Point4 *d_in, Point4 *d_out, int n, IcpState *st, bool stop_on_bad, hipStream_t s);
+hipError_t check_copy_frame(const Point4 *d_in, Point4 *d_out, int n, IcpState *st, bool stop_on_bad, ZeroWords zero, hipStream_t s);
 
 }
diff --git a/sage-icp_amd/csrc/kernels.hip b/sage-icp_amd/csrc/kernels.hip
--- a/sage-icp_amd/csrc/kernels.hip
+++ b/sage-icp_amd/csrc/kernels.hip
@@ -677,10 +677,11 @@
     (void)hipLaunchKernel(loop_kernel(lw, p.filter != 0), dim3(l.wgs), dim3(64 * l.nw), args, lds, s);
 #endif
 }
-void launch_loop_solve(const LoopParams &l, const P2pParams &x, hipStream_t s) {
+void launch_loop_solve(const LoopParams &l, const P2pParams &x, const StateMirror &m, hipStream_t s) {
     SolveArgs a;
     a.L = l;
     a.X = x;
+    a.M = m;
     if (l.copies == kChainReplicas) hipLaunchKernelGGL(k_loop_solve<kChainReplicas>, dim3(1), dim3(64), 0, s, a);
     else hipLaunchKernelGGL(k_loop_solve<kLoopReplicas>, dim3(1), dim3(64), 0, s, a);
 }
diff --git a/sage-icp_amd/csrc/loop_kernel.h b/sage-icp_amd/csrc/loop_kernel.h
--- a/sage-icp_amd/csrc/loop_kernel.h
+++ b/sage-icp_amd/csrc/loop_kernel.h
@@ -82,7 +82,7 @@
     if (const int al = lane_now(); al < kLoopPoseCopies) st_agent(&sh->pose[al][24], (tag << 32) | 2ull);
 }
 template <int COPIES>
-__device__ __forceinline__ unsigned loop_finish_iteration(const LoopParams &L, const P2pParams &X, SolveLds &m, int it,
+__device__ __forceinline__ unsigned loop_finish_iteration(const LoopParams &L, const P2pParams &X, const StateMirror &M, SolveLds &m, int it,
                                                           unsigned long long &xg) {
     LoopShared *sh = L.sh;
     IcpState *st = L.st;
@@ -203,29 +203,37 @@
         for (int c = 0; c < kLoopPoseCopies; c += 2)
             st_agent(&sh->pose[c + (pl >> 5)][gl], (tag << 32) | word);
     }
-    if (lane == 0) {
-        if (it < kHistory) st->n_corr[it] = static_cast<uint32_t>(S[kCount]);
-        if (overflow) st->acc_overflow = 1;
-        if (exchange_failed) st->exchange_failed = 1;
-        if (done) {
-#pragma unroll
-            for (int i = 0; i < 7; ++i) st->T[i] = Tn[i];
-#pragma unroll
-            for (int i = 0; i < 9; ++i) st->R[i] = Rn[i];
-            st->last_step_norm = nrm;
-            st->iter = it + 1;
-            st->done = 1;
-            st->converged = (converged && !exchange_failed) ? 1 : 0;
-        }
-    }
-    if (done && lane == 1) {
-#pragma unroll
-        for (int i = 0; i < 7; ++i) st->T_icp[i] = Tn[i];
+    auto leave = [&](IcpState *to) {
+        if (lane == 0) {
+            if (it < kHistory) to->n_corr[it] = static_cast<uint32_t>(S[kCount]);
+            if (overflow) to->acc_overflow = 1;
+            if (exchange_failed) to->exchange_failed = 1;
+            if (done) {
+#pragma unroll
+                for (int i = 0; i < 7; ++i) to->T[i] = Tn[i];
+#pragma unroll
+                for (int i = 0; i < 9; ++i) to->R[i] = Rn[i];
+                to->last_step_norm = nrm;
+                to->iter = it + 1;
+                to->done = 1;
+                to->converged = (converged && !exchange_failed) ? 1 : 0;
+            }
+        }
+        if (done && lane == 1) {
+#pragma unroll
+            for (int i = 0; i < 7; ++i) to->T_icp[i] = Tn[i];
+        }
+        if (done && lane < kNumSums) to->sums[lane] = S[lane];
+    };
+    leave(st);
+    if (M.st) leave(M.st);
+    if (done && M.st) {
+        asm volatile("s_waitcnt vmcnt(0)" ::: "memory");
+        if (lane == 0) *M.epoch_word = L.epoch;
     }
     if (L.progress && lane == 0)
         __hip_atomic_store(&L.progress->word, (static_cast<unsigned long long>(done ? 1u : 0u) << 32) | static_cast<unsigned long long>(it + 1),
                            __ATOMIC_RELAXED, __HIP_MEMORY_SCOPE_SYSTEM);
-    if (done && lane < kNumSums) st->sums[lane] = S[lane];
     LOOP_STAMP_SOLVER(it, 3);
     return done;
 }
@@ -233,6 +241,7 @@
 struct SolveArgs {
     LoopParams L;
     P2pParams X;
+    StateMirror M;
 };
 template <int COPIES>
 __global__ __launch_bounds__(64) void k_loop_solve(SolveArgs A) {
@@ -261,7 +270,7 @@
         auto ka = __builtin_amdgcn_kernarg_segment_ptr();
         asm volatile("" : "+s"(ka));
         const SolveArgs &K = *(const SolveArgs *)(ka);
-        if (loop_finish_iteration<COPIES>(K.L, K.X, m, it, xg)) return;
+        if (loop_finish_iteration<COPIES>(K.L, K.X, K.M, m, it, xg)) return;
     }
 }
 
@@ -308,8 +317,9 @@
         P2pParams X{};
         X.nranks = 1;
         unsigned long long xg = 0ull;
+        const StateMirror none{nullptr, nullptr};
         for (int it = 0;; ++it)
-            if (loop_finish_iteration<kLoopReplicas>(L, X, m, it, xg)) return;
+            if (loop_finish_iteration<kLoopReplicas>(L, X, none, m, it, xg)) return;
     }
 #endif
 
diff --git a/sage-icp_amd/csrc/sageicp_types.h b/sage-icp_amd/csrc/sageicp_types.h
--- a/sage-icp_amd/csrc/sageicp_types.h
+++ b/sage-icp_amd/csrc/sageicp_types.h
@@ -81,7 +81,8 @@
 
 struct IcpProgress {
     unsigned long long word;
-    unsigned long long pad_[7];
+    unsigned long long final_epoch;
+    unsigned long long pad_[6];
 };
 
 constexpr int kMaxRanks = 8;
diff --git a/sage-icp_amd/csrc/sort.hip b/sage-icp_amd/csrc/sort.hip
--- a/sage-icp_amd/csrc/sort.hip
+++ b/sage-icp_amd/csrc/sort.hip
@@ -1,5 +1,7 @@
 #include <hip/hip_runtime.h>
+#include <algorithm>
 #include <cstring>
+#include <utility>
 
 #include <rocprim/rocprim.hpp>
 
@@ -16,6 +18,34 @@
     return v;
 }
 
+__device__ __forceinline__ void refuse_non_finite(const Point4 &f, IcpState *st, int stop_on_bad) {
+    if (!(fabs(f.x) <= 1.7976931348623157e308 && fabs(f.y) <= 1.7976931348623157e308 &&
+          fabs(f.z) <= 1.7976931348623157e308 && fabs(f.l) <= 1.7976931348623157e308)) {
+        st->bad_input = 1;
+        if (stop_on_bad) {
+            st->done = 1;
+            if (IcpProgress *pg = st->progress)
+                __hip_atomic_store(&pg->word, 1ull << 32, __ATOMIC_RELAXED, __HIP_MEMORY_SCOPE_SYSTEM);
+        }
+    }
+}
+template <bool APPLY_POSE>
+__device__ __forceinline__ uint32_t morton_key(const Point4 &f, const IcpState *st, double voxel_size) {
+    double x = f.x, y = f.y, z = f.z;
+    if (APPLY_POSE) {
+        const double *R = st->R;
+        const double *T = st->T;
+        x = R[0] * f.x + R[1] * f.y + R[2] * f.z + T[4];
+        y = R[3] * f.x + R[4] * f.y + R[5] * f.z + T[5];
+        z = R[6] * f.x + R[7] * f.y + R[8] * f.z + T[6];
+    }
+    const int cx = static_cast<int>(x / voxel_size) + 512;
+    const int cy = static_cast<int>(y / voxel_size) + 512;
+    const int cz = static_cast<int>(z / voxel_size) + 512;
+    return spread10(static_cast<uint32_t>(cx)) | (spread10(static_cast<uint32_t>(cy)) << 1) |
+           (spread10(static_cast<uint32_t>(cz)) << 2);
+}
+
 template <bool APPLY_POSE>
 __global__ __launch_bounds__(256) void k_morton_keys(const Point4 *pts, int n, IcpState *st, int stop_on_bad,
                                                      double voxel_size, uint32_t *keys,
@@ -23,28 +53,8 @@
     const int i = blockIdx.x * 256 + threadIdx.x;
     if (i >= n) return;
     const Point4 f = pts[i];
-    if (!(fabs(f.x) <= 1.7976931348623157e308 && fabs(f.y) <= 1.7976931348623157e308 &&
-          fabs(f.z) <= 1.7976931348623157e308 && fabs(f.l) <= 1.7976931348623157e308)) {
-        st->bad_input = 1;
-        if (stop_on_bad) {
-            st->done = 1;
-            if (IcpProgress *pg = st->progress)
-                __hip_atomic_store(&pg->word, 1ull << 32, __ATOMIC_RELAXED, __HIP_MEMORY_SCOPE_SYSTEM);
-        }
-    }
-    double x = f.x, y = f.y, z = f.z;
-    if (APPLY_POSE) {
-        const double *R = st->R;
-        const double *T = st->T;
-        x = R[0] * f.x + R[1] * f.y + R[2] * f.z + T[4];
-        y = R[3] * f.x + R[4] * f.y + R[5] * f.z + T[5];
-        z = R[6] * f.x + R[7] * f.y + R[8] * f.z + T[6];
-    }
-    const int cx = static_cast<int>(x / voxel_size) + 512;
-    const int cy = static_cast<int>(y / voxel_size) + 512;
-    const int cz = static_cast<int>(z / voxel_size) + 512;
-    keys[i] = spread10(static_cast<uint32_t>(cx)) | (spread10(static_cast<uint32_t>(cy)) << 1) |
-              (spread10(static_cast<uint32_t>(cz)) << 2);
+    refuse_non_finite(f, st, stop_on_bad);
+    keys[i] = morton_key<APPLY_POSE>(f, st, voxel_size);
     vals[i] = static_cast<uint32_t>(i);
 }
 
@@ -55,38 +65,204 @@
     out[i] = in[perm[i]];
 }
 
-__global__ __launch_bounds__(256) void k_check_copy(const Point4 *pts, int n, IcpState *st, int stop_on_bad, Point4 *out) {
+__global__ __launch_bounds__(256) void k_check_copy(const Point4 *pts, int n, IcpState *st, int stop_on_bad, Point4 *out, ZeroWords zero) {
     const int i = blockIdx.x * 256 + threadIdx.x;
+    for (unsigned j = static_cast<unsigned>(i); j < zero.n; j += gridDim.x * 256u) zero.words[j] = 0ull;
     if (i >= n) return;
     const Point4 f = pts[i];
-    if (!(fabs(f.x) <= 1.7976931348623157e308 && fabs(f.y) <= 1.7976931348623157e308 &&
-          fabs(f.z) <= 1.7976931348623157e308 && fabs(f.l) <= 1.7976931348623157e308)) {
-        st->bad_input = 1;
-        if (stop_on_bad) {
-            st->done = 1;
-            if (IcpProgress *pg = st->progress)
-                __hip_atomic_store(&pg->word, 1ull << 32, __ATOMIC_RELAXED, __HIP_MEMORY_SCOPE_SYSTEM);
-        }
-    }
+    refuse_non_finite(f, st, stop_on_bad);
     out[i] = f;
 }
-hipError_t check_copy_frame(const Point4 *d_in, Point4 *d_out, int n, IcpState *st, bool stop_on_bad, hipStream_t s) {
-    if (n <= 0) return hipSuccess;
-    hipLaunchKernelGGL(k_check_copy, dim3((n + 255) / 256), dim3(256), 0, s, d_in, n, st, stop_on_bad ? 1 : 0, d_out);
+hipError_t check_copy_frame(const Point4 *d_in, Point4 *d_out, int n, IcpState *st, bool stop_on_bad, ZeroWords zero, hipStream_t s) {
+    if (n <= 0) return zero.n ? hipMemsetAsync(zero.words, 0, sizeof(unsigned long long) * zero.n, s) : hipSuccess;
+    hipLaunchKernelGGL(k_check_copy, dim3((n + 255) / 256), dim3(256), 0, s, d_in, n, st, stop_on_bad ? 1 : 0, d_out, zero);
     return hipGetLastError();
 }
 
-size_t sort_temp_bytes(int n) {
+constexpr int kFsThreads = 1024, kFsWaves = kFsThreads / 64;
+constexpr int kFsRounds = kFrameSortTile / kFsThreads;
+constexpr uint32_t kFsNoKey = 0xFFFFFFFFu;
+constexpr int kFsSlots = 2 * kFrameSortTile;
+
+template <bool APPLY_POSE>
+__global__ __launch_bounds__(kFsThreads) void k_frame_keys(const Point4 *pts, int n, IcpState *st, int stop_on_bad, double voxel_size,
+                                                           uint32_t *keys, uint32_t *vals, uint32_t *counts, ZeroWords zero) {
+    __shared__ uint32_t hist[kFrameSortDigits];
+    const unsigned t = threadIdx.x, tiles = gridDim.x;
+    for (unsigned j = blockIdx.x * static_cast<unsigned>(kFsThreads) + t; j < zero.n; j += tiles * static_cast<unsigned>(kFsThreads)) zero.words[j] = 0ull;
+    if (t < static_cast<unsigned>(kFrameSortDigits)) hist[t] = 0u;
+    __syncthreads();
+#pragma unroll
+    for (int r = 0; r < kFsRounds; ++r) {
+        const int i = static_cast<int>(blockIdx.x) * kFrameSortTile + r * kFsThreads + static_cast<int>(t);
+        if (i >= n) continue;
+        const Point4 f = pts[i];
+        refuse_non_finite(f, st, stop_on_bad);
+        const uint32_t key = morton_key<APPLY_POSE>(f, st, voxel_size);
+        keys[i] = key;
+        vals[i] = static_cast<uint32_t>(i);
+        __hip_atomic_fetch_add(&hist[key & 255u], 1u, __ATOMIC_RELAXED, __HIP_MEMORY_SCOPE_WORKGROUP);
+    }
+    __syncthreads();
+    if (t >= static_cast<unsigned>(kFrameSortDigits)) return;
+    counts[static_cast<size_t>(blockIdx.x) * kFrameSortDigits + t] = hist[t];
+    for (unsigned p = 1; p < static_cast<unsigned>(kFrameSortPasses); ++p)
+        counts[(static_cast<size_t>(p) * tiles + blockIdx.x) * kFrameSortDigits + t] = 0u;
+}
+
+__device__ __forceinline__ uint32_t fs_exclusive_scan(uint32_t v, uint32_t *wsum) {
+    const unsigned lane = threadIdx.x & 63u, wave = threadIdx.x >> 6;
+    uint32_t inc = v;
+#pragma unroll
+    for (unsigned o = 1; o < 64u; o <<= 1) {
+        const uint32_t u = __shfl_up(inc, o);
+        if (lane >= o) inc += u;
+    }
+    if (lane == 63u) wsum[wave] = inc;
+    __syncthreads();
+    uint32_t before = 0u;
+    for (unsigned w = 0; w < wave; ++w) before += wsum[w];
+    return inc - v + before;
+}
+
+template <bool LAST>
+__global__ __launch_bounds__(kFsThreads) void k_frame_pass(const uint32_t *kin, const uint32_t *vin, uint32_t *kout, uint32_t *vout, int n,
+                                                           int shift, const uint32_t *counts, uint32_t *next, const Point4 *in, Point4 *out) {
+    __shared__ uint32_t cnt[kFsWaves][kFrameSortDigits];
+    __shared__ uint32_t col_before[kFrameSortDigits], col_total[kFrameSortDigits], wsum[kFsWaves];
+    __shared__ uint32_t slot_key[LAST ? 1 : kFsSlots], slot_cnt[LAST ? 1 : kFsSlots];
+    const unsigned t = threadIdx.x, lane = t & 63u, wave = t >> 6, tiles = gridDim.x, tile = blockIdx.x;
+    uint32_t key[kFsRounds], val[kFsRounds], rank[kFsRounds];
+    const int first = static_cast<int>(tile) * kFrameSortTile + static_cast<int>(wave) * (kFrameSortTile / kFsWaves) + static_cast<int>(lane);
+#pragma unroll
+    for (int r = 0; r < kFsRounds; ++r) {
+        const int i = first + r * 64;
+        key[r] = i < n ? kin[i] : kFsNoKey;
+        val[r] = i < n ? vin[i] : 0u;
+    }
+    uint32_t before = 0u, total = 0u;
+    {
+        const unsigned d = t & 255u;
+#pragma unroll 8
+        for (unsigned k = t >> 8; k < tiles; k += 4u) {
+            const uint32_t c = counts[static_cast<size_t>(k) * kFrameSortDigits + d];
+            total += c;
+            before += k < tile ? c : 0u;
+        }
+    }
+#pragma unroll
+    for (int w = t >> 8; w < kFsWaves; w += 4) cnt[w][t & 255u] = 0u;
+    if (t < static_cast<unsigned>(kFrameSortDigits)) {
+        col_before[t] = 0u;
+        col_total[t] = 0u;
+    }
+    if (!LAST)
+        for (unsigned j = t; j < static_cast<unsigned>(kFsSlots); j += static_cast<unsigned>(kFsThreads)) {
+            slot_key[j] = kFsNoKey;
+            slot_cnt[j] = 0u;
+        }
+    __syncthreads();
+    __hip_atomic_fetch_add(&col_before[t & 255u], before, __ATOMIC_RELAXED, __HIP_MEMORY_SCOPE_WORKGROUP);
+    __hip_atomic_fetch_add(&col_total[t & 255u], total, __ATOMIC_RELAXED, __HIP_MEMORY_SCOPE_WORKGROUP);
+#pragma unroll
+    for (int r = 0; r < kFsRounds; ++r) {
+        const bool valid = first + r * 64 < n;
+        const uint32_t d = (key[r] >> shift) & 255u;
+        unsigned long long peers = __ballot(valid);
+#pragma unroll
+        for (int b = 0; b < 8; ++b) {
+            const bool bit = (d >> b) & 1u;
+            const unsigned long long set = __ballot(bit);
+            peers &= bit ? set : ~set;
+        }
+        const int leader = valid ? __ffsll(static_cast<long long>(peers)) - 1 : static_cast<int>(lane);
+        uint32_t start = 0u;
+        if (valid && static_cast<int>(lane) == leader)
+            start = __hip_atomic_fetch_add(&cnt[wave][d], static_cast<uint32_t>(__popcll(peers)), __ATOMIC_RELAXED, __HIP_MEMORY_SCOPE_WORKGROUP);
+        start = __shfl(start, leader);
+        rank[r] = start + static_cast<uint32_t>(__popcll(peers & ((1ull << lane) - 1ull)));
+    }
+    __syncthreads();
+    {
+        const bool digit = t < static_cast<unsigned>(kFrameSortDigits);
+        uint32_t at = fs_exclusive_scan(digit ? col_total[t] : 0u, wsum);
+        if (digit) {
+            at += col_before[t];
+#pragma unroll
+            for (int w = 0; w < kFsWaves; ++w) {
+                const uint32_t c = cnt[w][t];
+                cnt[w][t] = at;
+                at += c;
+            }
+        }
+    }
+    __syncthreads();
+#pragma unroll
+    for (int r = 0; r < kFsRounds; ++r) {
+        if (first + r * 64 >= n) continue;
+        const uint32_t place = cnt[wave][(key[r] >> shift) & 255u] + rank[r];
+        if (place >= static_cast<uint32_t>(n) || val[r] >= static_cast<uint32_t>(n)) continue;
+        if (LAST) {
+            vout[place] = val[r];
+            out[place] = in[val[r]];
+        } else {
+            kout[place] = key[r];
+            vout[place] = val[r];
+            const uint32_t k = ((place / static_cast<uint32_t>(kFrameSortTile)) << 8) | ((key[r] >> (shift + 8)) & 255u);
+            uint32_t h = (k * 0x9E3779B1u) >> 20;
+            for (;;) {
+                const uint32_t seen = atomicCAS(&slot_key[h], kFsNoKey, k);
+                if (seen == kFsNoKey || seen == k) break;
+                h = (h + 1u) & static_cast<uint32_t>(kFsSlots - 1);
+            }
+            __hip_atomic_fetch_add(&slot_cnt[h], 1u, __ATOMIC_RELAXED, __HIP_MEMORY_SCOPE_WORKGROUP);
+        }
+    }
+    if (LAST) return;
+    __syncthreads();
+    for (unsigned j = t; j < static_cast<unsigned>(kFsSlots); j += static_cast<unsigned>(kFsThreads)) {
+        const uint32_t k = slot_key[j];
+        if (k != kFsNoKey && (k >> 8) < tiles)
+            __hip_atomic_fetch_add(&next[static_cast<size_t>(k >> 8) * kFrameSortDigits + (k & 255u)], slot_cnt[j], __ATOMIC_RELAXED, __HIP_MEMORY_SCOPE_AGENT);
+    }
+}
+static_assert(kFsSlots == 4096 && kFrameSortDigits == 256 && kFrameSortPasses * 8 >= 30 && kFsRounds == 2 && kFsWaves == 16,
+              "k_frame_pass is written for these");
+
+static hipError_t sort_frame_own(const Point4 *d_in, Point4 *d_out, int n, IcpState *st, bool apply_pose, bool stop_on_bad, double voxel_size,
+                                 uint32_t *keys, uint32_t *vals, uint32_t *counts, ZeroWords zero, hipStream_t s) {
+    const unsigned tiles = static_cast<unsigned>(frame_sort_tiles(n));
+    const size_t per_pass = static_cast<size_t>(tiles) * kFrameSortDigits;
+    uint32_t *ka = keys + n, *va = vals + n, *kb = keys, *vb = vals;
+    if (apply_pose)
+        hipLaunchKernelGGL(k_frame_keys<true>, dim3(tiles), dim3(kFsThreads), 0, s, d_in, n, st, stop_on_bad ? 1 : 0, voxel_size, ka, va, counts, zero);
+    else
+        hipLaunchKernelGGL(k_frame_keys<false>, dim3(tiles), dim3(kFsThreads), 0, s, d_in, n, st, stop_on_bad ? 1 : 0, voxel_size, ka, va, counts, zero);
+    for (int p = 0; p + 1 < kFrameSortPasses; ++p) {
+        hipLaunchKernelGGL(k_frame_pass<false>, dim3(tiles), dim3(kFsThreads), 0, s, ka, va, kb, vb, n, 8 * p, counts + p * per_pass,
+                           counts + (p + 1) * per_pass, static_cast<const Point4 *>(nullptr), static_cast<Point4 *>(nullptr));
+        std::swap(ka, kb);
+        std::swap(va, vb);
+    }
+    hipLaunchKernelGGL(k_frame_pass<true>, dim3(tiles), dim3(kFsThreads), 0, s, ka, va, kb, vb, n, 8 * (kFrameSortPasses - 1),
+                       counts + (kFrameSortPasses - 1) * per_pass, static_cast<uint32_t *>(nullptr), d_in, d_out);
+    return hipGetLastError();
+}
+
+static size_t rocprim_temp_bytes(int n) {
     size_t bytes = 0;
     uint32_t *k = nullptr;
     (void)rocprim::radix_sort_pairs(nullptr, bytes, k, k, k, k, static_cast<unsigned>(n), 0, 30);
     return bytes;
 }
+size_t sort_temp_bytes(int n) { return std::max(rocprim_temp_bytes(n), frame_sort_own_bytes(n)); }
 
 hipError_t sort_frame(const Point4 *d_in, Point4 *d_out, int n, IcpState *st, bool apply_pose, bool stop_on_bad,
                       double voxel_size, uint32_t *keys, uint32_t *vals, void *temp,
-                      size_t temp_bytes, hipStream_t s) {
-    if (n <= 0) return hipSuccess;
+                      size_t temp_bytes, int impl, ZeroWords zero, hipStream_t s) {
+    if (n <= 0) return zero.n ? hipMemsetAsync(zero.words, 0, sizeof(unsigned long long) * zero.n, s) : hipSuccess;
+    if (frame_sort_own_path(impl, n) && frame_sort_own_bytes(n) <= temp_bytes)
+        return sort_frame_own(d_in, d_out, n, st, apply_pose, stop_on_bad, voxel_size, keys, vals, static_cast<uint32_t *>(temp), zero, s);
     const int grid = (n + 255) / 256;
     if (apply_pose)
         hipLaunchKernelGGL(k_morton_keys<true>, dim3(grid), dim3(256), 0, s, d_in, n, st, stop_on_bad ? 1 : 0,
@@ -98,6 +274,7 @@
                                              static_cast<unsigned>(n), 0, 30, s);
     if (e != hipSuccess) return e;
     hipLaunchKernelGGL(k_gather, dim3(grid), dim3(256), 0, s, d_in, vals + n, n, d_out);
+    if (zero.n) return hipMemsetAsync(zero.words, 0, sizeof(unsigned long long) * zero.n, s);
     return hipGetLastError();
 }
 
```
